# ut-vision/Rot-MVGaze

Measured on AMD Instinct MI355X. Metric: multi-view samples/sec (fwd+bwd), BxVx3x224x224, higher is better.
Workload: dtype f32; 1 GPU; C3: ResNet-50, V=4, B=128 per GPU, 3x224x224, fwd+loss+bwd; backbone=ResNet-50, views=4, batch_per_gpu=128, global_batch=128, image=3x224x224, parallelism=dp1, weights=random init, seed 0 (kaiming-normal convs, default Linear), rccl_ranks=1, step_launch=eager: every kernel queued from Python

## Files before the change

include/rotmvgaze.h:

```cpp
#ifndef ROTMVGAZE_H
#define ROTMVGAZE_H

#include <stddef.h>
#include <stdint.h>

#ifdef __cplusplus
extern "C" {
#endif

#define MVG_ABI_VERSION 13

int mvg_abi_version(void);
const char *mvg_last_error(void);
int mvg_device_cus(void);
int mvg_set_scratch(void *ptr, size_t bytes, void *stream);
size_t mvg_scratch_bytes(void);
void *mvg_stream_create_low_priority(void);
int mvg_set_reserved_cus(int n);

enum {
  MVG_K_CONV_FPROP = 0, MVG_K_CONV_DGRAD = 1, MVG_K_CONV_WGRAD = 2, MVG_K_WGRAD_REDUCE = 3,
  MVG_K_BN_FINALIZE = 4, MVG_K_BN_APPLY = 5, MVG_K_BN_BWD_REDUCE = 6, MVG_K_BN_BWD_APPLY = 7,
  MVG_K_POOL = 8, MVG_K_LAYOUT = 9, MVG_K_LINEAR_FPROP = 10, MVG_K_LINEAR_DGRAD = 11,
  MVG_K_LINEAR_WGRAD = 12, MVG_K_ROTCAT = 13, MVG_K_COLSUM = 14, MVG_K_LOSS = 15,
// ... 288 lines not shown
                                        int ho, int wo, float *s1, float *s2, float *dgamma, float *dbeta,
                                        int accumulate, float *workspace, void *stream);
int mvg_bn_relu_maxpool_bwd_apply_bf16(const uint16_t *g_pooled, const uint8_t *argmax, const uint16_t *y,
                                       const float *mean, const float *invstd, const float *gamma,
                                       const float *scale, const float *shift, const float *s1,
                                       const float *s2, int groups, int n_per_group, int h, int w, int c,
                                       int ho, int wo, uint16_t *dy, void *stream);
int mvg_bn_eval_bwd_bf16(const uint16_t *g, const uint16_t *act, const uint8_t *relu_bits, const uint16_t *y,
                         const float *relu_scale, const float *relu_shift, const float *gamma, const float *running_mean,
                         const float *running_var, float eps, int groups, int64_t rows_per_group, int c, uint16_t *dy,
                         uint16_t *dz_out, float *dgamma, float *dbeta, int accumulate, float *workspace, void *stream);
int mvg_bn_relu_maxpool_eval_bwd_bf16(const uint16_t *g_pooled, const uint8_t *argmax, const uint16_t *y, const float *scale,
                                      const float *shift, const float *gamma, const float *running_mean,
                                      const float *running_var, float eps, int groups, int n_per_group, int h, int w,
                                      int c, int ho, int wo, uint16_t *dy, float *dgamma, float *dbeta, int accumulate,
                                      float *workspace, void *stream);
int mvg_avgpool_fwd_bf16(const uint16_t *x, float *y, int n, int hw, int c, void *stream);
int mvg_avgpool_bwd_bf16(const float *dy, uint16_t *dx, int n, int hw, int c, void *stream);
int mvg_nchw_to_nhwc8_bf16(const float *src, uint16_t *dst, int n, int c, int h, int w, void *stream);
int mvg_preprocess_u8hwc_resize_bf16(const uint8_t *src, uint16_t *dst, int n, int h, int w, int oh, int ow, float mean0,
                                     float mean1, float mean2, float std0, float std1, float std2, int swap_rb,
                                     void *stream);

int mvg_split_f32(const float *x, void *out_sp, int64_t n, float scale, void *stream);
int mvg_merge_sp(const void *x_sp, float *out, int64_t n, float inv_scale, void *stream);
int mvg_split_weights(const mvg_conv_desc *d, const float *w, void *w_krsc_sp, void *w_crsk_sp, float *stat2, void *items_dev,
                      void *stream);
int mvg_weights_prep_batch(const void *items_dev, int n, int mode, int blocks_per_item , void *stream);
int mvg_conv_stats_partials_split(const mvg_conv_desc *d, int32_t *rows_per_partial);
int mvg_conv_fprop_split(const mvg_conv_desc *d, const void *x_sp, const float *x_sinv, const void *w_sp, const float *w_sinv,
                         float *y, float *stats, void *stream);
int mvg_conv_fprop_split_affine(const mvg_conv_desc *d, const void *x_sp, const float *x_sinv, const void *w_sp, const float *w_sinv,
                                void *out, int out_sp, const float *scale, const float *shift, const void *residual,
                                int residual_sp, int relu, void *stream);
int mvg_conv_fprop_split_affine_ranged(const mvg_conv_desc *d, const void *x_sp, const float *x_sinv, const void *w_sp,
                                       const float *w_sinv, void *out, int out_sp, const float *scale, const float *shift,
                                       const void *residual, int residual_sp, int relu, uint32_t *range_word, void *stream);
int mvg_split_f32_ranged(const float *x, void *out_sp, int64_t n, float scale, uint32_t *range_word, void *stream);
int mvg_conv_dgrad_split(const mvg_conv_desc *d, const void *dy_sp, const float *dy_sinv, const void *w_crsk_sp,
                         const float *w_sinv, float *dx, const float *addend, const void *relu_mask_sp, void *stream);
int mvg_bn_apply_split(const float *y, const float *scale, const float *shift, const void *residual, int residual_sp,
                       const float *res_scale, const float *res_shift, int relu, void *out_sp, uint8_t *relu_bits,
                       int groups, int64_t rows_per_group, int c, void *stream);
int mvg_bn_bwd_reduce_split(const float *g, const uint8_t *relu_bits, const float *y, const float *mean, const float *invstd,
                            const float *relu_scale, const float *relu_shift, int groups, int64_t rows_per_group, int c,
                            float *s1, float *s2, float *dgamma, float *dbeta, int accumulate, float *workspace,
                            float *dz_out, float *mx, const float *gamma, float *dy_sinv, void *stream);
int mvg_bn_bwd_apply_split(const float *g, const float *y, const float *mean, const float *invstd, const float *gamma,
                           const float *s1, const float *s2, const float *relu_scale, const float *relu_shift,
                           int groups, int64_t rows_per_group, int c, void *dy_sp, const float *mx, float *dy_sinv,
                           int dy_sinv_ready, void *stream);
int mvg_bn_relu_maxpool_fwd_split(const float *y, const float *scale, const float *shift, void *pooled_sp,
                                  uint8_t *argmax, int groups, int n_per_group, int h, int w, int c, int ho, int wo,
                                  void *stream);
int mvg_avgpool_fwd_split(const void *x_sp, float *y, int n, int hw, int c, void *stream);
int mvg_act_scales(const void *items_dev, int n, float *slots, int n_slots, void *stream);
int mvg_bn_apply_split_scaled(const float *y, const float *scale, const float *shift, const void *residual, int residual_sp,
                              const float *res_scale, const float *res_shift, const float *res_sinv, int relu, void *out_sp,
                              const float *out_sinv, uint8_t *relu_bits, int groups, int64_t rows_per_group, int c,
                              void *stream);
int mvg_bn_relu_maxpool_fwd_split_scaled(const float *y, const float *scale, const float *shift, void *pooled_sp,
                                         const float *pooled_sinv, uint8_t *argmax, int groups, int n_per_group, int h, int w,
                                         int c, int ho, int wo, void *stream);
int mvg_avgpool_fwd_split_scaled(const void *x_sp, const float *x_sinv, float *y, int n, int hw, int c, void *stream);
int mvg_conv_dgrad_bn_partials_split(const mvg_conv_desc *d);
int mvg_conv_dgrad_split_bnreduce(const mvg_conv_desc *d, const void *dy_sp, const float *dy_sinv, const void *w_crsk_sp,
                                  const float *w_sinv, float *dx, const float *addend, const float *bn_y, const uint8_t *bn_bits,
                                  const float *bn_mean, const float *bn_invstd, const float *relu_scale, const float *relu_shift,
                                  float *partials, float *s1, float *s2, float *dgamma, float *dbeta, int accumulate,
                                  float *mx, const float *bn_gamma, float *dx_dy_sinv, void *stream);
int mvg_conv_dgrad_split_bnapply_bnreduce(const mvg_conv_desc *d, void *dy_sp, const float *dy_sinv, const float *dz, const float *y,
                                          const float *mean, const float *invstd, const float *gamma, const float *un_s1,
                                          const float *un_s2, int64_t rows_per_group, const void *w_crsk_sp, const float *w_sinv,
                                          float *dx, const float *addend, const float *bn_y, const uint8_t *bn_bits,
                                          const float *bn_mean, const float *bn_invstd, const float *relu_scale,
                                          const float *relu_shift, float *partials, float *s1, float *s2, float *dgamma, float *dbeta,
                                          int accumulate, float *mx, const float *bn_gamma, float *dx_dy_sinv, void *stream);
int mvg_conv_fprop_split_stages(const mvg_conv_desc *d);
int mvg_conv_dgrad_split_stages(const mvg_conv_desc *d, int fused_reduce);
int mvg_conv_fprop_split_bnapply(const mvg_conv_desc *d, void *out_sp, const float *out_sinv, const float *bn_y, const float *scale,
                                 const float *shift, const void *residual, int residual_sp, const float *res_scale,
                                 const float *res_shift, const float *res_sinv, uint8_t *relu_bits, const void *w_sp,
                                 const float *w_sinv, float *y, float *stats, void *stream);
int mvg_stem_rowwindow_split(const float *x_nhwc4, void *xw_sp, int64_t images, int h, int w, void *stream);
int mvg_stem_rowwindow_split_nchw(const float *x_nchw, void *xw_sp, int64_t images, int h, int w, void *stream);
int mvg_stem_fprop_split(const mvg_conv_desc *d, const void *xw_sp, const void *w_sp, const float *w_sinv, float *y, float *stats,
                         void *stream);
int mvg_stem_wgrad_splits_split(const mvg_conv_desc *d);
int mvg_stem_wgrad_split(const mvg_conv_desc *d, const void *xw_sp, const void *dy_sp, const float *dy_sinv, float *dw_rw,
                         float *workspace, int splits, int accumulate, void *stream);
int mvg_bn_relu_maxpool_bwd_reduce_split(const float *g_pooled, const uint8_t *argmax, const float *y, const float *mean,
                                         const float *invstd, const float *scale, const float *shift, int groups,
                                         int n_per_group, int h, int w, int c, int ho, int wo, float *s1, float *s2,
                                         float *dgamma, float *dbeta, int accumulate, float *workspace, float *mx, const float *gamma,
                                         float *dy_sinv, void *stream);
int mvg_bn_relu_maxpool_bwd_apply_split(const float *g_pooled, const uint8_t *argmax, const float *y, const float *mean,
                                        const float *invstd, const float *gamma, const float *scale, const float *shift,
                                        const float *s1, const float *s2, int groups, int n_per_group, int h, int w, int c,
                                        int ho, int wo, void *dy_sp, const float *mx, float *dy_sinv, int dy_sinv_ready, void *stream);
int mvg_conv_wgrad_splits_split(const mvg_conv_desc *d);
int mvg_conv_wgrad_split_tile(const mvg_conv_desc *d, int32_t *bm, int32_t *bn, int32_t *incremental);
int mvg_conv_wgrad_split(const mvg_conv_desc *d, const void *x_sp, const void *dy_sp, const float *dy_sinv, float *dw,
                         float *workspace, int splits, int accumulate, void *stream);
int mvg_conv_wgrad_split_slabs(const mvg_conv_desc *d, const void *x_sp, const void *dy_sp, const float *dy_sinv, float *workspace,
                               int splits, void *stream);
int mvg_conv_wgrad_split_xs(const mvg_conv_desc *d, const void *x_sp, const float *x_sinv, const void *dy_sp, const float *dy_sinv,
                            float *dw, float *workspace, int splits, int accumulate, void *stream);
int mvg_conv_wgrad_split_slabs_xs(const mvg_conv_desc *d, const void *x_sp, const float *x_sinv, const void *dy_sp,
                                  const float *dy_sinv, float *workspace, int splits, void *stream);
int mvg_wgrad_reduce_batch(const float *const *host_slabs, float *const *host_dw, const int64_t *host_n, const int32_t *host_splits,
                           const int32_t *host_accumulate, int n, void *stream);

int mvg_absmax_multi(const float *const *host_ptrs, const int64_t *host_counts, float *const *host_out_slots, int n, void *stream);
int mvg_fuse_build_split(const float *img_feat, const float *feat, const float *rel, const int32_t *row_img, const int32_t *row_src_f,
                         const int32_t *row_src_h, void *xf_sp, void *xh_sp, const float *am_img, const float *am_feat,
                         float *xf_sinv, float *xh_sinv, int rows, int cf, int nvec, void *stream);
int mvg_fuse_unbuild(const float *dxh, const float *dxn, const float *rel, const int32_t *seg, const int32_t *vi, float *dfeat, float *da,
                     int da_accumulate, int segments, int views, int dirs, int batch, int cf, int nvec, float *absmax, void *stream);
int mvg_linear_fprop_split(int rows, int fin, int fout, const void *x_sp, const float *x_sinv, const void *w_sp, const float *w_sinv,
                           const float *bias, int relu, void *out, int out_sp, float *out_sinv, const float *bias_absmax,
                           float *out_absmax, void *stream);
int mvg_linear_dgrad_split(int rows, int fin, int fout, const void *dy_sp, const float *dy_sinv, const void *wt_sp, const float *w_sinv,
                           float *dx, const float *addend, const void *relu_mask_sp, float *out_absmax, void *stream);
int mvg_linear_wgrad_split(int rows, int fin, int fout, const void *x_sp, const float *x_sinv, const void *dy_sp, const float *dy_sinv,
                           float *dw, float *workspace, int splits, int accumulate, void *stream);
int mvg_split_colsum(const float *g, int rows, int cols, const float *absmax, void *out_sp, float *out_sinv, float *db, int accumulate,
                     void *stream);

typedef struct mvg_session mvg_session;
typedef struct {
  int32_t depth;
  int32_t num_iter;
  int32_t views, batch;
  int32_t height, width;
  int32_t share_weights, ignore_rotmat;
  int32_t split;
  int32_t raw_u8;
  int32_t in_h, in_w, input_bgr;
} mvg_session_cfg;

int mvg_session_create(const mvg_session_cfg *cfg, mvg_session **out);
#define MVG_SESSION_FP32 0
#define MVG_SESSION_BF16 1
int mvg_session_create_ex(const mvg_session_cfg *cfg, int32_t compute, mvg_session **out);
int mvg_session_compute(const mvg_session *s);
void mvg_session_destroy(mvg_session *s);
int mvg_session_num_tensors(const mvg_session *s);
const char *mvg_session_tensor_name(const mvg_session *s, int i);
int64_t mvg_session_tensor_numel(const mvg_session *s, int i);
size_t mvg_session_workspace_bytes(const mvg_session *s);
int mvg_session_launches(const mvg_session *s);
int mvg_session_num_steps(const mvg_session *s);
const char *mvg_session_step_name(const mvg_session *s, int i);
int mvg_session_bind(mvg_session *s, const void *const *host_tensor_ptrs, void *workspace, size_t bytes, void *stream);
int mvg_session_forward(mvg_session *s, const void *const *host_view_ptrs, const float *rot, float *img_feat, float *lifted,
                        float *feats, float *preds, void *stream);
int mvg_session_num_range_units(const mvg_session *s);
const char *mvg_session_range_unit_name(const mvg_session *s, int i);
int mvg_session_set_range_record(mvg_session *s, uint32_t *record_dev);

#ifdef __cplusplus
}
#endif
#endif
```

rot-mvgaze_amd/_lib.py:

```python
from __future__ import annotations

import ctypes as C
import os

_HERE = os.path.dirname(os.path.abspath(__file__))
LIB_PATH = os.path.join(_HERE, "csrc", "librotmvgaze_hip.so")

K_FAMILIES = 18
ABI_VERSION = 13
SESSION_FP32, SESSION_BF16 = 0, 1
ADAM_MAX_SEGMENTS = 16


class ConvDesc(C.Structure):
    _fields_ = [(n, C.c_int32) for n in
                ("groups", "n", "h", "w", "cin", "cout", "r", "s", "stride", "pad", "ho", "wo")]

    @classmethod
    def make(cls, groups, n, h, w, cin, cout, k, stride, pad):
        ho = (h + 2 * pad - k) // stride + 1
        wo = (w + 2 * pad - k) // stride + 1
        return cls(groups, n, h, w, cin, cout, k, k, stride, pad, ho, wo)

    @classmethod
# ... 25 lines not shown
                ("lanes_per_group", C.c_int32), ("slices", C.c_int32), ("partials_per_slice", C.c_int32), ("scratch_floats", C.c_int64)]


class ProfEntry(C.Structure):
    _fields_ = [("launches", C.c_int64), ("ms", C.c_double), ("flops", C.c_double), ("bytes", C.c_double)]


class SessionCfg(C.Structure):
    _fields_ = [(n, C.c_int32) for n in
                ("depth", "num_iter", "views", "batch", "height", "width", "share_weights", "ignore_rotmat", "split", "raw_u8",
                 "in_h", "in_w", "input_bgr")]


_P = C.c_void_p
_I = C.c_int
_I64 = C.c_int64
_F = C.c_float
_D = C.POINTER(ConvDesc)

SIGNATURES = {
    "mvg_abi_version": (_I, []),
    "mvg_last_error": (C.c_char_p, []),
    "mvg_device_cus": (_I, []),
    "mvg_set_scratch": (_I, [_P, C.c_size_t, _P]),
    "mvg_scratch_bytes": (C.c_size_t, []),
    "mvg_set_reserved_cus": (_I, [_I]),
    "mvg_stream_create_low_priority": (_P, []),
    "mvg_prof_enable": (_I, [_I]),
    "mvg_prof_reset": (_I, []),
    "mvg_prof_collect": (_I, [C.POINTER(ProfEntry)]),
    "mvg_prof_family_name": (C.c_char_p, [_I]),
    "mvg_conv_fprop": (_I, [_D, _P, _P, _P, _P, _I, _P, _P]),
    "mvg_conv_fprop_affine": (_I, [_D, _P, _P, _P, _P, _P, _P, _I, _P]),
    "mvg_conv_stats_partials": (_I, [_D, C.POINTER(C.c_int32)]),
    "mvg_conv_dgrad": (_I, [_D, _P, _P, _P, _P, _P, _P]),
    "mvg_conv_wgrad": (_I, [_D, _P, _P, _P, _P, _I, _I, _P]),
    "mvg_conv_wgrad_splits": (_I, [_D]),
    "mvg_conv_plan_query": (_I, [_D, _I, C.c_size_t, C.POINTER(ConvPlan)]),
    "mvg_bn_plan_query": (_I, [_I, _I, _I, _I64, _I, _I, _I, _I, _I, C.c_size_t, C.POINTER(BnPlan)]),
    "mvg_conv_wgrad_tile": (_I, [_D, C.POINTER(C.c_int32), C.POINTER(C.c_int32), C.POINTER(C.c_int32)]),
    "mvg_linear_wgrad": (_I, [_P, _P, _P, _P, _I, _I, _I, _P, _I, _I, _P]),
    "mvg_fuser_fprop": (_I, [_P, _P, _P, _P, _P, _P, _P, _I, _P, _I, _I, _I, _I, _I, _I, _P, C.c_size_t, _P]),
    "mvg_fuser_wgrad": (_I, [_P, _P, _P, _P, _P, _P, _P, _P, _I, _I, _I, _I, _I, _I, _P, _I, _I, _P]),
    "mvg_linear_workspace_floats": (C.c_size_t, [_I, _I, _I]),
    "mvg_linear_fprop": (_I, [_P, _P, _P, _I, _P, _I, _I, _I, _P, C.c_size_t, _P]),
    "mvg_linear_dgrad": (_I, [_P, _P, _P, _P, _P, _I, _I, _I, _P, C.c_size_t, _P]),
    "mvg_bn_finalize": (_I, [_P, _I, _I, _I, _I64, _I, _P, _P, _P, _P, _F, _F, _P, _P, _P, _P, _P]),
    "mvg_bn_eval_affine": (_I, [_I, _I, _P, _P, _P, _P, _F, _P, _P, _P]),
    "mvg_bn_eval_affine_batch": (_I, [_P, _I, _I, _F, _P]),
    "mvg_bn_apply": (_I, [_P, _P, _P, _P, _P, _P, _I, _P, _I, _I64, _I, _P]),
    "mvg_bn_bwd_reduce": (_I, [_P, _P, _P, _P, _P, _P, _P, _I, _I64, _I, _P, _P, _P, _P, _I, _P, _P, _P]),
    "mvg_split_f32": (_I, [_P, _P, _I64, _F, _P]),
    "mvg_merge_sp": (_I, [_P, _P, _I64, _F, _P]),
    "mvg_split_weights": (_I, [_D, _P, _P, _P, _P, _P, _P]),
    "mvg_weights_prep_batch": (_I, [_P, _I, _I, _I, _P]),
    "mvg_conv_stats_partials_split": (_I, [_D, C.POINTER(C.c_int32)]),
    "mvg_conv_fprop_split": (_I, [_D, _P, _P, _P, _P, _P, _P, _P]),
    "mvg_conv_fprop_split_affine": (_I, [_D, _P, _P, _P, _P, _P, _I, _P, _P, _P, _I, _I, _P]),
    "mvg_conv_dgrad_split": (_I, [_D, _P, _P, _P, _P, _P, _P, _P, _P]),
    "mvg_bn_apply_split": (_I, [_P, _P, _P, _P, _I, _P, _P, _I, _P, _P, _I, _I64, _I, _P]),
    "mvg_bn_bwd_apply_split": (_I, [_P, _P, _P, _P, _P, _P, _P, _P, _P, _I, _I64, _I, _P, _P, _P, _I, _P]),
    "mvg_bn_bwd_reduce_split": (_I, [_P, _P, _P, _P, _P, _P, _P, _I, _I64, _I, _P, _P, _P, _P, _I, _P, _P, _P, _P, _P, _P]),
    "mvg_bn_relu_maxpool_fwd_split": (_I, [_P, _P, _P, _P, _P, _I, _I, _I, _I, _I, _I, _I, _P]),
    "mvg_avgpool_fwd_split": (_I, [_P, _P, _I, _I, _I, _P]),
    "mvg_act_scales": (_I, [_P, _I, _P, _I, _P]),
    "mvg_bn_apply_split_scaled": (_I, [_P, _P, _P, _P, _I, _P, _P, _P, _I, _P, _P, _P, _I, _I64, _I, _P]),
    "mvg_bn_relu_maxpool_fwd_split_scaled": (_I, [_P, _P, _P, _P, _P, _P, _I, _I, _I, _I, _I, _I, _I, _P]),
    "mvg_avgpool_fwd_split_scaled": (_I, [_P, _P, _P, _I, _I, _I, _P]),
    "mvg_conv_wgrad_split_xs": (_I, [_D, _P, _P, _P, _P, _P, _P, _I, _I, _P]),
    "mvg_conv_wgrad_split_slabs_xs": (_I, [_D, _P, _P, _P, _P, _P, _I, _P]),
    "mvg_stem_rowwindow_split": (_I, [_P, _P, _I64, _I, _I, _P]),
    "mvg_stem_rowwindow_split_nchw": (_I, [_P, _P, _I64, _I, _I, _P]),
    "mvg_stem_fprop_split": (_I, [_D, _P, _P, _P, _P, _P, _P]),
    "mvg_stem_wgrad_splits_split": (_I, [_D]),
    "mvg_stem_wgrad_split": (_I, [_D, _P, _P, _P, _P, _P, _I, _I, _P]),
    "mvg_bn_relu_maxpool_bwd_reduce_split": (_I, [_P, _P, _P, _P, _P, _P, _P, _I, _I, _I, _I, _I, _I, _I, _P, _P, _P, _P, _I, _P, _P, _P, _P, _P]),
    "mvg_bn_relu_maxpool_bwd_apply_split": (_I, [_P, _P, _P, _P, _P, _P, _P, _P, _P, _P, _I, _I, _I, _I, _I, _I, _I, _P, _P, _P, _I, _P]),
    "mvg_conv_dgrad_bn_partials_split": (_I, [_D]),
    "mvg_conv_dgrad_split_bnreduce": (_I, [_D, _P, _P, _P, _P, _P, _P, _P, _P, _P, _P, _P, _P, _P, _P, _P, _P, _P, _I, _P, _P, _P, _P]),
    "mvg_conv_dgrad_split_bnapply_bnreduce": (_I, [_D] + [_P] * 9 + [_I64] + [_P] * 15 + [_I, _P, _P, _P, _P]),
    "mvg_conv_fprop_split_stages": (_I, [_D]),
    "mvg_conv_dgrad_split_stages": (_I, [_D, _I]),
    "mvg_conv_fprop_split_bnapply": (_I, [_D] + [_P] * 6 + [_I] + [_P] * 9),
    "mvg_conv_wgrad_splits_split": (_I, [_D]),
    "mvg_conv_wgrad_split_tile": (_I, [_D, C.POINTER(C.c_int32), C.POINTER(C.c_int32), C.POINTER(C.c_int32)]),
    "mvg_conv_wgrad_split": (_I, [_D, _P, _P, _P, _P, _P, _I, _I, _P]),
    "mvg_conv_wgrad_split_slabs": (_I, [_D, _P, _P, _P, _P, _I, _P]),
    "mvg_wgrad_reduce_batch": (_I, [C.POINTER(C.c_void_p), C.POINTER(C.c_void_p), C.POINTER(C.c_int64), C.POINTER(C.c_int32),
                                    C.POINTER(C.c_int32), _I, _P]),
    "mvg_bn_apply_bits": (_I, [_P, _P, _P, _P, _P, _P, _P, _P, _I, _I64, _I, _P]),
    "mvg_bn_bwd_reduce_bits": (_I, [_P, _P, _P, _P, _P, _I, _I64, _I, _P, _P, _P, _P, _I, _P, _P, _P]),
    "mvg_bn_apply_bits_bf16": (_I, [_P, _P, _P, _P, _P, _P, _P, _P, _I, _I64, _I, _P]),
    "mvg_bn_bwd_reduce_bits_bf16": (_I, [_P, _P, _P, _P, _P, _I, _I64, _I, _P, _P, _P, _P, _I, _P, _P, _P]),
    "mvg_bn_bwd_workspace_floats": (C.c_size_t, [_I, _I64, _I]),
    "mvg_bn_bwd_apply": (_I, [_P, _P, _P, _P, _P, _P, _P, _P, _P, _P, _I, _I64, _I, _P, _P, _P]),
    "mvg_maxpool3x3s2_fwd": (_I, [_P, _P, _P, _I, _I, _I, _I, _I, _I, _P]),
    "mvg_maxpool3x3s2_bwd": (_I, [_P, _P, _P, _I, _I, _I, _I, _I, _I, _P]),
    "mvg_bn_relu_maxpool_fwd": (_I, [_P, _P, _P, _P, _P, _I, _I, _I, _I, _I, _I, _I, _P]),
    "mvg_bn_relu_maxpool_bwd_reduce": (_I, [_P, _P, _P, _P, _P, _P, _P, _I, _I, _I, _I, _I, _I, _I, _P, _P, _P, _P, _I, _P,
                                            _P]),
    "mvg_bn_relu_maxpool_bwd_apply": (_I, [_P, _P, _P, _P, _P, _P, _P, _P, _P, _P, _I, _I, _I, _I, _I, _I, _I, _P, _P]),
    "mvg_bn_eval_bwd": (_I, [_P, _P, _P, _P, _P, _P, _P, _P, _P, _F, _I, _I64, _I, _P, _P, _P, _P, _I, _P, _P]),
    "mvg_bn_eval_bwd_workspace_floats": (C.c_size_t, [_I, _I64, _I]),
    "mvg_bn_relu_maxpool_eval_bwd": (_I, [_P, _P, _P, _P, _P, _P, _P, _P, _F, _I, _I, _I, _I, _I, _I, _I, _P, _P, _P, _I, _P,
                                          _P]),
    "mvg_avgpool_fwd": (_I, [_P, _P, _I, _I, _I, _P]),
    "mvg_avgpool_bwd": (_I, [_P, _P, _I, _I, _I, _P]),
    "mvg_nchw_to_nhwc4": (_I, [_P, _P, _I, _I, _I, _I, _P]),
    "mvg_nhwc4_to_nchw": (_I, [_P, _P, _I, _I, _I, _I, _P]),
    "mvg_preprocess_u8hwc": (_I, [_P, _P, _I, _I, _I, _F, _F, _F, _F, _F, _F, _I, _P]),
    "mvg_gaze_lp_loss": (_I, [_P, _P, _I, _I, _P, _P, _P]),
    "mvg_preprocess_u8hwc_resize": (_I, [_P, _P, _I, _I, _I, _I, _I, _F, _F, _F, _F, _F, _F, _I, _P]),
    "mvg_multi_erase_nchw": (_I, [_P, _P, _P, _I, _I, _I, _I, _I, _P]),
    "mvg_augment_u8hwc": (_I, [_P, _P, _P, _P, _P, _P, _P, _I, _I, _I, _I, _F, _F, _F, _F, _F, _F, _I, _P]),
    "mvg_augment_u8hwc_bf16": (_I, [_P, _P, _P, _P, _P, _P, _P, _I, _I, _I, _I, _F, _F, _F, _F, _F, _F, _I, _P]),
    "mvg_rotation_matrix_2d": (_I, [_P, _P, _I, _I, _P]),
    "mvg_relative_rotation": (_I, [_P, _P, _P, _P, _I, _I, _I, _P]),
    "mvg_rotcat_fwd": (_I, [_P, _P, _P, _P, _P, _P, _I, _I, _I, _I, _P]),
    "mvg_rotcat_bwd": (_I, [_P, _P, _P, _P, _I, _I, _I, _I, _P]),
    "mvg_rotcat_ext_fwd": (_I, [_P, _P, _P, _P, _P, _P, _P, _I, _I, _I, _I, _I, _P]),
    "mvg_rotcat_ext_bwd": (_I, [_P, _I, _P, _P, _P, _I, _I, _I, _I, _P]),
    "mvg_ibn_scales": (_I, [_P, _P, _P, _P, _P, _I, _F, _F, _P, _I, _I, _I, _P]),
    "mvg_paircat_fwd": (_I, [_P, _P, _P, _P, _P, _P, _P, _I, _I, _I, _P]),
    "mvg_paircat_bwd": (_I, [_P, _P, _P, _P, _P, _P, _I, _I, _I, _P]),
    "mvg_segment_sum": (_I, [_P, _I64, _I, _P, _P, _I, _I, _I, _I, _P]),
    "mvg_axpby": (_I, [_P, _P, _F, _F, _I64, _P]),
    "mvg_scale_by": (_I, [_P, _P, _P, _I64, _P]),
    "mvg_linear_skinny_fwd": (_I, [_P, _P, _P, _P, _I, _I, _I, _P]),
    "mvg_linear_skinny_bwd": (_I, [_P, _P, _P, _P, _P, _P, _P, _I, _I, _I, _I, _P, _P]),
    "mvg_adam_step": (_I, [_P, _P, _P, _P, _I64, _F, _F, _F, _F, _F, _I, _P]),
    "mvg_gaze_angular_loss": (_I, [_P, _P, _I, _F, _P, _I, _P, _P, _P]),
    "mvg_gaze_angular_loss_multi": (_I, [_P, _P, _I, _I, _I, C.POINTER(C.c_float), _P, _P, _P]),
    "mvg_adam_step_dev": (_I, [_P, _P, _P, _P, _I64, _P, _P, _F, _F, _F, _F, _P]),
    "mvg_adam_step_segments": (_I, [_P, _P, _P, _P, _I64, C.POINTER(C.c_int64), C.POINTER(C.c_float), C.POINTER(C.c_int32), _I, _P]),
    "mvg_adam_step_segments_dev": (_I, [_P, _P, _P, _P, _I64, C.POINTER(C.c_int64), C.POINTER(C.c_float), C.POINTER(C.c_int32), _I, _P, _I, _P,
                                        _P]),
    "mvg_absmax_multi": (_I, [C.POINTER(C.c_void_p), C.POINTER(C.c_int64), C.POINTER(C.c_void_p), _I, _P]),
    "mvg_fuse_build_split": (_I, [_P, _P, _P, _P, _P, _P, _P, _P, _P, _P, _P, _P, _I, _I, _I, _P]),
    "mvg_fuse_unbuild": (_I, [_P, _P, _P, _P, _P, _P, _P, _I, _I, _I, _I, _I, _I, _I, _P, _P]),
    "mvg_linear_fprop_split": (_I, [_I, _I, _I, _P, _P, _P, _P, _P, _I, _P, _I, _P, _P, _P, _P]),
    "mvg_linear_dgrad_split": (_I, [_I, _I, _I, _P, _P, _P, _P, _P, _P, _P, _P, _P]),
    "mvg_linear_wgrad_split": (_I, [_I, _I, _I, _P, _P, _P, _P, _P, _P, _I, _I, _P]),
    "mvg_split_colsum": (_I, [_P, _I, _I, _P, _P, _P, _P, _I, _P]),
    "mvg_cast_weights_bf16": (_I, [_D, _P, _I, _P, _P, _P]),
    "mvg_conv_fprop_bf16": (_I, [_D, _P, _P, _P, _P, _I, _P, _P]),
    "mvg_conv_stats_partials_bf16": (_I, [_D, C.POINTER(C.c_int32)]),
    "mvg_conv_fprop_bf16_affine": (_I, [_D, _P, _P, _P, _P, _P, _P, _I, _P]),
    "mvg_conv_dgrad_bf16": (_I, [_D, _P, _P, _P, _P, _P, _P]),
    "mvg_conv_dgrad_bn_partials_bf16": (_I, [_D]),
    "mvg_conv_dgrad_bf16_bnreduce": (_I, [_D, _P, _P, _P, _P, _P, _P, _P, _P, _P, _P, _P, _P, _P, _P, _P, _I, _P]),
    "mvg_conv_wgrad_bf16": (_I, [_D, _P, _P, _P, _P, _I, _I, _P]),
    "mvg_stem_rowwindow_bf16": (_I, [_P, _P, _I64, _I, _I, _P]),
    "mvg_stem_fprop_bf16": (_I, [_D, _P, _P, _P, _P, _P]),
    "mvg_stem_wgrad_splits_bf16": (_I, [_D]),
    "mvg_stem_wgrad_bf16": (_I, [_D, _P, _P, _P, _P, _I, _I, _P]),
    "mvg_conv_wgrad_splits_bf16": (_I, [_D]),
    "mvg_conv_wgrad_bf16_slabs": (_I, [_D, _P, _P, _P, _I, _P]),
    "mvg_conv_plan_query_bf16": (_I, [_D, _I, C.POINTER(ConvPlan)]),
    "mvg_conv_wgrad_tile_bf16": (_I, [_D, _I, C.POINTER(C.c_int32), C.POINTER(C.c_int32), C.POINTER(C.c_int32)]),
    "mvg_linear_fprop_mixed": (_I, [_P, _P, _P, _I, _P, _I, _I, _I, _P]),
    "mvg_linear_dgrad_mixed": (_I, [_P, _P, _P, _P, _P, _I, _I, _I, _P]),
    "mvg_linear_wgrad_mixed": (_I, [_P, _P, _P, _P, _I, _I, _I, _P, _I, _I, _P]),
    "mvg_bn_apply_bf16": (_I, [_P, _P, _P, _P, _P, _P, _I, _P, _I, _I64, _I, _P]),
    "mvg_bn_bwd_reduce_bf16": (_I, [_P, _P, _P, _P, _P, _P, _P, _I, _I64, _I, _P, _P, _P, _P, _I, _P, _P, _P]),
    "mvg_bn_bwd_apply_bf16": (_I, [_P, _P, _P, _P, _P, _P, _P, _P, _P, _P, _I, _I64, _I, _P, _P, _P]),
    "mvg_bn_relu_maxpool_fwd_bf16": (_I, [_P, _P, _P, _P, _P, _I, _I, _I, _I, _I, _I, _I, _P]),
# ... 62 lines not shown
```

rot-mvgaze_amd/backbone.py:

```python
from __future__ import annotations

import enum
import math
import os
from dataclasses import dataclass
from typing import Callable, Dict, List, NamedTuple, Optional

import numpy as np
import torch

from . import ops
from ._lib import ConvDesc
from .arch import RANGE_OVER_BITS, BackboneSpec, ConvSpec, backbone_spec, range_unit_names

Tensor = torch.Tensor
BN_EPS, BN_MOMENTUM = 1e-5, 0.1
IMAGE_MEAN, IMAGE_STD = (0.485, 0.456, 0.406), (0.229, 0.224, 0.225)


BN_APPLY_DGRAD_MAX_COUT = 512


def bn_apply_dgrad_eligible(c: ConvSpec, *, split: bool, trained: bool, fused_in: bool, carries_reduce: bool,
                            need_dimg: bool = False) -> bool:
    return bool(split and trained and not need_dimg and fused_in and carries_reduce
                and c.k == 1 and c.stride == 1 and c.pad == 0 and c.cin in (64, 128)
                and c.cout % 32 == 0 and c.cout <= BN_APPLY_DGRAD_MAX_COUT)


def bn_apply_dgrad_units(spec: BackboneSpec, *, split: bool = True, bf16: bool = False, training: bool = True,
                         need_dimg: bool = False, fuse_bn_split: bool = True, enabled: bool = True) -> List[str]:
    on = enabled and split and not bf16 and fuse_bn_split
    nb = len(spec.blocks)
    return [blk.convs[-1].name for bi, blk in reversed(list(enumerate(spec.blocks)))
            if bn_apply_dgrad_eligible(blk.convs[-1], split=on, trained=training, fused_in=bi < nb - 1,
                                       carries_reduce=len(blk.convs) > 1, need_dimg=need_dimg)]


BN_APPLY_FPROP_MAX_CIN = 512


def bn_apply_fprop_eligible(producer: ConvSpec, consumer: ConvSpec, *, split: bool, trained: bool, residual: bool = True,
                            relu: bool = True, single_stage: bool = True) -> bool:
    return bool(split and trained and residual and relu and single_stage
                and consumer.k == 1 and consumer.stride == 1 and consumer.pad == 0 and consumer.cout in (64, 128)
                and consumer.cin == producer.cout and consumer.cin % 32 == 0 and consumer.cin <= BN_APPLY_FPROP_MAX_CIN)


def bn_apply_fprop_pairs(spec: BackboneSpec, *, split: bool = True, bf16: bool = False, training: bool = True, enabled: bool = True,
                         single_stage: Optional[Callable[[ConvSpec], bool]] = None) -> List[tuple]:
    on = enabled and split and not bf16
    return [(a.convs[-1].name, b.convs[0].name) for a, b in zip(spec.blocks[:-1], spec.blocks[1:])
            if bn_apply_fprop_eligible(a.convs[-1], b.convs[0], split=on, trained=training,
                                       single_stage=True if single_stage is None else single_stage(b.convs[0]))]


class GradSink:

    def view(self, p: torch.nn.Parameter) -> Tensor:
        raise NotImplementedError

    def wants(self, p: torch.nn.Parameter) -> bool:
        return True

    def accumulate(self, p: torch.nn.Parameter) -> bool:
        raise NotImplementedError

    def publish(self, ps: List[torch.nn.Parameter]) -> None:
        raise NotImplementedError


class Family(enum.Enum):
    FP32 = 0
    SPLIT = 1
    BF16 = 2


class Call(NamedTuple):
    V: int
    B: int
    H: int
    W: int
    training: bool
    keep_tape: bool
    bf16: bool
    split: bool
    sp: bool
    stem_rw: bool
    taped: bool
    guard: Optional[str]
    range_live: bool
    need_dimg: bool
    boundary: int
    wprep: Optional[Dict[str, tuple]] = None
    act_sinv: Optional[Dict[str, Tensor]] = None
    train_step: Optional[bool] = None


def plan_call(spec: BackboneSpec, *, V: int, B: int, H: int, W: int, training: bool, keep_tape: bool, raw: bool = False,
              augment: bool = False, need_dimg: bool = False, boundary: int = -1, bf16: bool = False, split: bool = True,
              split_eval: bool = True, split_eval_guard: Optional[str] = None, stem_rowwindow: bool = True,
              batch_weight_prep: bool = True, bf16_fold_eval: bool = True, guard_scale: int = 1, tripped: bool = False,
              capturing: bool = False, train_step: Optional[bool] = None) -> Call:
    step = training if train_step is None else bool(train_step)
    if bf16 and raw and (step or keep_tape) and not (step and augment):
        raise NotImplementedError("raw uint8 input with the bf16 path is served for inference only (model.eval() under "
                                  "torch.no_grad()) and for training steps with model.input_augment (augment.TrainAugment; the "
                                  "identity augment for un-augmented steps): else normalise to fp32 NCHW first")
    biggest_view_elems = B * ((H + 3) // 4) * ((W + 3) // 4) * spec.blocks[0].convs[-1].cout
    split = split and 4 * biggest_view_elems * guard_scale < 0x7FFFFFF0
    infer = not (training or keep_tape or bf16)
    if split_eval_guard not in (None, "record", "fallback"):
        raise ValueError(f"split_eval_guard must be None, 'record' or 'fallback' (got {split_eval_guard!r})")
    guard = split_eval_guard if infer else None
    if guard == "fallback" and capturing:
        raise RuntimeError("split_eval_guard = 'fallback' reads the range record on the host and cannot run while the stream "
                           "is capturing: capture with 'record' and check overflowed() after the replay")
    if guard == "fallback" and tripped:
        split = False
    if bf16:
        ho, wo = (H - 1) // 2 + 1, W // 2
        stem_rw = (stem_rowwindow and training and W % 4 == 0 and (B * ho * (wo // 2)) % 64 == 0 and batch_weight_prep
                   and spec.stem.k == 7)
    else:
        stem_rw = (split and stem_rowwindow and training and not need_dimg and W % 2 == 0
                   and batch_weight_prep and 32 * B * H * (W // 2) * 4 < 0x7FFFFFF0)
    taped = training or keep_tape or (bf16 and not bf16_fold_eval)
    sp = split and not bf16 and (training or (infer and split_eval))
    return Call(V, B, H, W, training, keep_tape, bf16, split, sp, stem_rw, taped, guard,
                range_live=guard is not None and sp, need_dimg=need_dimg, boundary=boundary, train_step=step)


def unit_family(call: Call, c: ConvSpec) -> Family:
    if call.bf16:
        return Family.BF16
    if call.sp and (c.cin != 3 or call.stem_rw):
        return Family.SPLIT
    return Family.FP32


class _Apply(NamedTuple):
    y: Tensor
    scale: Tensor
    shift: Tensor
    residual: Optional[Tensor]
    residual_affine: Optional[tuple]
    bits: Optional[Tensor]


class _PendingDy(NamedTuple):
    dz: Tensor
    s1: Tensor
    s2: Tensor


class _FusedSums(NamedTuple):
    s1: Tensor
    s2: Tensor
    mx: Optional[Tensor] = None
    sinv: Optional[Tensor] = None


class _Pool(NamedTuple):
    argmax: Tensor
    scale: Tensor
    shift: Tensor
    ho: int
    wo: int
    hp: int
    wp: int


@dataclass(slots=True)
class _Unit:
    spec: Optional[ConvSpec] = None
    desc: Optional[ConvDesc] = None
    x_in: Optional[Tensor] = None
    y: Optional[Tensor] = None
    out: Optional[Tensor] = None
    mean: Optional[Tensor] = None
    invstd: Optional[Tensor] = None
    relu: bool = False
    rows: int = 0
    w: Optional[Tensor] = None
    trained: bool = True
    pool: Optional[_Pool] = None
    relu_affine: Optional[tuple] = None
    fused_s12: Optional[_FusedSums] = None
    relu_bits: Optional[Tensor] = None
    family: Family = Family.FP32
    stem_rw: bool = False


class _Fwd(NamedTuple):
    out: Tensor
    affine: Optional[tuple] = None
    pending: Optional[_Apply] = None


class Backbone:
    _guard_scale = 1
    _debug_units: Optional[list] = None

    def __init__(self, depth: int, params: Dict[str, Tensor], prefix: str = "_feat_extractor.0."):
        self.spec: BackboneSpec = backbone_spec(depth, prefix)
        self.p = params
        self.fc_dim = self.spec.fc_dim
        self.overlap_wgrad = True
        self.overlap_head = True
        self.wgrad_low_priority = True
        self.grad_streams: List[torch.cuda.Stream] = []
        self._wg_stream: Optional[torch.cuda.Stream] = None
        self._wg_low = True
        self.act_dtype = torch.float32
        self.relu_bits = True
        self.split = os.environ.get("MVG_SPLIT", "1") != "0"
        self.fuse_bn_split = True
        self.fuse_bn_apply_dgrad = True
        self.fuse_bn_apply_fprop = True
        self.stem_rowwindow = True
        self.split_eval = True
        self.split_eval_guard: Optional[str] = None
        self._range_record: Optional[Tensor] = None
        self._range_slot: Dict[str, int] = {n: i for i, n in enumerate(range_unit_names(depth, prefix))}
        self._range_tripped = False
        self.bf16_fold_eval = True
        self._wprep_infer_ok = False
        self._wk_cache: Dict[str, tuple] = {}
        self.batch_weight_prep = True
        self._wprep_state = None
        self._wprep_versions = None
        self._ascale_state = None
        self._wg_defer: Optional[list] = None
        self._last_call: Optional[Call] = None
        self._stem_w8 = None

    @property
    def bf16(self) -> bool:
        return self.act_dtype == torch.bfloat16

    @property
    def _split_now(self) -> bool:
        return self._last_call.split if self._last_call is not None else self.split

    @property
    def _stem_rw(self) -> bool:
        return self._last_call is not None and self._last_call.stem_rw

    @property
    def _act_sinv(self) -> Optional[Dict[str, Tensor]]:
        return self._last_call.act_sinv if self._last_call is not None else None

    def _prepare_weights(self, dev, family: Family, stem_rw: bool, reuse: bool = False) -> Dict[str, tuple]:
        mode = 0 if family is Family.BF16 else 1
        convs = [c for c in self.spec.all_convs() if not (mode == 1 and c.cin == 3 and not stem_rw)]
        key = (mode, stem_rw, str(dev), tuple(self.p[c.name + ".weight"].data_ptr() for c in convs))
        if self._wprep_state is None or self._wprep_state[0] != key:
            out, rows = {}, []
            wstat = torch.zeros(len(convs), 2, dtype=torch.float32, device=dev)
            self._stem_w8 = None
            for ci, c in enumerate(convs):
                wsrc = self.p[c.name + ".weight"]
                assert wsrc.is_contiguous(memory_format=torch.channels_last) or (c.k == 1 and wsrc.is_contiguous())
                rs = c.k * c.k
                if mode == 1 and c.cin == 3:
                    assert c.k == 7
                    self._stem_w8 = torch.zeros(c.cout, 7, 8, 4, dtype=torch.float32, device=dev)
                    wk = ops.sp_empty(c.cout, 7 * 32, device=dev)
                    wk.sinv = wstat[ci, 1:2]
                    out[c.name] = (wk, None)
                    rows.append([self._stem_w8.data_ptr(), wk.data_ptr(), 0, c.cout | (7 << 32), 32 | (32 << 32), wstat[ci].data_ptr()])
                    continue
                if mode == 0 and c.cin == 3 and stem_rw:
                    assert c.k == 7
                    self._stem_w8 = torch.zeros(2 * c.cout, 7, 16, 4, dtype=torch.float32, device=dev)
                    wk = torch.empty(2 * c.cout, 7, 1, 64, dtype=torch.bfloat16, device=dev)
                    out[c.name] = (wk, None)
                    rows.append([self._stem_w8.data_ptr(), wk.data_ptr(), 0, (2 * c.cout) | (7 << 32), 64 | (64 << 32), wstat[ci].data_ptr()])
                    continue
                if mode == 1:
                    wk = ops.sp_empty(c.cout, rs * c.cin, device=dev)
                    wt = ops.sp_empty(c.cin, rs * c.cout, device=dev)
                    wk.sinv = wt.sinv = wstat[ci, 1:2]
                    cin_pad = c.cin
                else:
                    cin_pad = 8 if c.cin == 3 else c.cin
                    wk = torch.empty(c.cout, c.k, c.k, cin_pad, dtype=torch.bfloat16, device=dev)
                    wt = None if c.cin == 3 else torch.empty(cin_pad, c.k, c.k, c.cout, dtype=torch.bfloat16, device=dev)
                out[c.name] = (wk, wt)
                rows.append([wsrc.data_ptr(), wk.data_ptr(), wt.data_ptr() if wt is not None else 0, c.cout | (rs << 32),
                             c.cin | (cin_pad << 32), wstat[ci].data_ptr()])
            table = torch.tensor(rows, dtype=torch.int64).to(dev)
            self._wprep_state = (key, out, table, len(rows), mode, wstat)
        elif (reuse and self._wprep_infer_ok and
              self._wprep_versions == tuple(self.p[c.name + ".weight"]._version for c in self.spec.all_convs())):
            return self._wprep_state[1]
        _, out, table, n, mode, wstat = self._wprep_state
        self._wprep_infer_ok = reuse
        if mode == 1:
            wstat.zero_()
            if self._stem_w8 is not None:
                self._stem_w8[:, :, 1:, :3].copy_(self.p[self.spec.stem.name + ".weight"].detach().permute(0, 2, 3, 1))
# ... 118 lines not shown
                self._debug_units.append((c.name, x, residual, y))
            return y
        ops.conv_fprop_affine(d, x, w, y, scale, shift, residual, relu)
        if not pool:
            return y
        pooled = self._pool_plain(y, G, N, d.ho, d.wo, c.cout)
        if call.range_live:
            return ops.split_f32_ranged(pooled, self._range_word(c))
        return ops.split_f32(pooled) if call.sp else pooled

    def _range_word(self, c: ConvSpec) -> Tensor:
        i = self._range_slot[c.name]
        return self._range_record[i:i + 1]

    @staticmethod
    def _pool_plain(a0: Tensor, G: int, N: int, h: int, w: int, c: int) -> Tensor:
        hp, wp_ = (h + 2 - 3) // 2 + 1, (w + 2 - 3) // 2 + 1
        x = torch.empty(G, N, hp, wp_, c, dtype=torch.float32, device=a0.device)
        argmax = torch.empty(G, N, hp, wp_, c, dtype=torch.uint8, device=a0.device)
        ops.maxpool_fwd(a0, x, argmax, G * N, h, w, c, hp, wp_)
        return x

    @staticmethod
    def _stats_partials(c: ConvSpec, d: ConvDesc, family: Family, stem_rw: bool):
        if family is Family.BF16:
            if stem_rw:
                P, rpp = ops.conv_stats_partials(ConvDesc.make(d.groups, d.n, d.ho, d.wo // 2, 64, 2 * c.cout, 1, 1, 0), True)
                return 2 * P, rpp
            return ops.conv_stats_partials(d, True)
        if family is Family.SPLIT:
            if stem_rw:
                return ops.conv_stats_partials_split(ConvDesc.make(d.groups, d.n, d.ho, d.wo, 32, c.cout, 1, 1, 0))
            return ops.conv_stats_partials_split(d)
        return ops.conv_stats_partials(d, False)

    def _unit_fwd(self, call: Call, c: ConvSpec, x: Tensor, H: int, W: int, *, relu: bool, residual: Optional[Tensor] = None,
                  tape: Optional[list] = None, pool: bool = False, residual_affine=None, defer_apply: bool = False,
                  next_conv: Optional[ConvSpec] = None, pending_apply: Optional[_Apply] = None) -> _Fwd:
        family = unit_family(call, c)
        stem_rw = c.cin == 3 and call.stem_rw
        G, N, training, keep = call.V, call.B, call.training, tape is not None
        d = ConvDesc.make(G, N, H, W, (8 if family is Family.BF16 else 4) if c.cin == 3 else c.cin, c.cout, c.k, c.stride, c.pad)
        assert pending_apply is None or (family is Family.SPLIT and not stem_rw)
        assert not stem_rw or call.wprep is not None
        w, w_t = self._conv_weights(call, c, d, family, keep)
        rows = N * d.ho * d.wo
        partials = self._stats_partials(c, d, family, stem_rw) if training else None
        y, stats = self._conv_fwd(c, d, family, stem_rw, x, w, pending_apply, partials)
        mean, invstd, scale, shift = self._bn_fwd_stats(c, G, rows, stats, partials)
        out = bits = pool_rec = handed = None
        if defer_apply:
            assert not relu and residual is None and not pool
        elif pool:
            assert relu and residual is None
            out, pool_rec = self._stem_tail(call, c, d, y, scale, shift)
            if self._debug_units is not None and not keep and not training:
                self._debug_units.append((c.name, x, y, out))
        else:
            out, bits, handed = self._apply_fwd(call, c, d, family, y, scale, shift, relu, residual, residual_affine, keep, next_conv)
        if keep:
            tape.append(_Unit(spec=c, desc=d, x_in=x, y=y, out=None if pool else out, mean=mean, invstd=invstd, relu=relu,
                              rows=rows, w=w if family is Family.FP32 else w_t, trained=training, family=family, stem_rw=stem_rw,
                              relu_affine=(scale, shift) if (relu and residual is None and not pool) else None,
                              pool=pool_rec, relu_bits=bits))
        return _Fwd(y, affine=(scale, shift)) if defer_apply else _Fwd(out, pending=handed)

    def _conv_fwd(self, c: ConvSpec, d: ConvDesc, family: Family, stem_rw: bool, x: Tensor, w: Tensor,
                  pending_apply: Optional[_Apply], partials: Optional[tuple]):
        dev = x.device
        y = torch.empty(d.groups, d.n, d.ho, d.wo, c.cout, dtype=self.act_dtype, device=dev)
        stats = None
        if partials is not None:
            stats = torch.empty(d.groups, partials[0], 2, c.cout, dtype=torch.float32, device=dev)
        if family is Family.BF16:
            if stem_rw:
                ops.stem_fprop_bf16(d, x, w, y, stats)
            else:
                ops.conv_fprop(d, x, w, y, None, False, stats)
        elif family is Family.SPLIT:
            if stem_rw:
                ops.stem_fprop_split(d, x, w, y, stats)
            elif pending_apply is not None:
                p = pending_apply
                ops.conv_fprop_split_bnapply(d, x, p.y, p.scale, p.shift, p.residual, w, y, stats, p.residual_affine, p.bits)
            else:
                ops.conv_fprop_split(d, x, w, y, stats)
        else:
            ops.conv_fprop(d, x, w, y, None, False, stats)
        return y, stats

    def _bn_fwd_stats(self, c: ConvSpec, G: int, rows: int, stats: Optional[Tensor], partials: Optional[tuple]):
        gamma, beta = self.p[c.bn + ".weight"].detach(), self.p[c.bn + ".bias"].detach()
        rm, rv = self.p[c.bn + ".running_mean"], self.p[c.bn + ".running_var"]
        mean, invstd, scale, shift = torch.empty(4, G, c.cout, dtype=torch.float32, device=gamma.device)
        if partials is not None:
            P, rpp = partials
            ops.bn_finalize(stats, G, P, rpp, rows, c.cout, gamma, beta, rm, rv, BN_MOMENTUM, BN_EPS, mean, invstd,
                            scale, shift)
        else:
            ops.bn_eval_affine(G, c.cout, gamma, beta, rm, rv, BN_EPS, scale, shift)
        return mean, invstd, scale, shift

    def _apply_fwd(self, call: Call, c: ConvSpec, d: ConvDesc, family: Family, y: Tensor, scale: Tensor, shift: Tensor, relu: bool,
                   residual: Optional[Tensor], residual_affine, keep: bool, next_conv: Optional[ConvSpec]):
        G, rows = d.groups, d.n * d.ho * d.wo
        if call.sp:
            out = ops.sp_empty(G, d.n, d.ho, d.wo, c.cout, device=y.device)
            out.sinv = call.act_sinv[c.name]
            want_bits = keep and relu and residual is not None
            if (next_conv is not None and self.fuse_bn_apply_fprop
                    and bn_apply_fprop_eligible(c, next_conv, split=family is Family.SPLIT, trained=call.training,
                                                residual=residual is not None, relu=relu)
                    and ops.conv_fprop_split_stages(ConvDesc.make(G, d.n, d.ho, d.wo, next_conv.cin, next_conv.cout, 1, 1, 0)) == 1):
                bits = torch.empty(G * rows * c.cout // 4, dtype=torch.uint8, device=y.device) if want_bits else None
                return out, bits, _Apply(y, scale, shift, residual, residual_affine, bits)
            bits = ops.bn_apply_split(y, scale, shift, residual, relu, out, G, rows, c.cout, residual_affine, want_bits=want_bits)
            return out, bits, None
        out = torch.empty_like(y) if keep else y
        if keep and relu and residual is not None and self.relu_bits:
            return out, ops.bn_apply_bits(y, scale, shift, residual, out, G, rows, c.cout, residual_affine), None
        ops.bn_apply(y, scale, shift, residual, relu, out, G, rows, c.cout, residual_affine)
        return out, None, None

    def _stem_tail(self, call: Call, c: ConvSpec, d: ConvDesc, y: Tensor, scale: Tensor, shift: Tensor):
        G, N = y.shape[0], y.shape[1]
        hp, wp_ = (d.ho + 2 - 3) // 2 + 1, (d.wo + 2 - 3) // 2 + 1
        argmax = torch.empty(G, N, hp, wp_, c.cout, dtype=torch.uint8, device=y.device)
        if call.sp:
            out = ops.sp_empty(G, N, hp, wp_, c.cout, device=y.device)
            out.sinv = call.act_sinv[c.name]
            ops.bn_relu_maxpool_fwd_split(y, scale, shift, out, argmax, G, N, d.ho, d.wo, c.cout, hp, wp_)
        else:
            out = torch.empty(G, N, hp, wp_, c.cout, dtype=self.act_dtype, device=y.device)
            ops.bn_relu_maxpool_fwd(y, scale, shift, out, argmax, G, N, d.ho, d.wo, c.cout, hp, wp_)
        return out, _Pool(argmax, scale, shift, d.ho, d.wo, hp, wp_)

    def _input_layout(self, call: Call, imgs: List[Tensor], input_bgr: bool, augment=None) -> Tensor:
        V, B, H, W, dev, bf = call.V, call.B, call.H, call.W, imgs[0].device, call.bf16
        raw = imgs[0].dtype == torch.uint8
        direct = call.stem_rw and (not raw or (bf and augment is not None))
        if direct and bf:
            x0 = torch.empty(V, B, H, W // 4, 64, dtype=self.act_dtype, device=dev)
        elif direct:
            x0 = ops.sp_empty(V, B, H, W // 2, 32, device=dev)
            x0.sinv = None
        else:
            x0 = torch.empty(V, B, H, W, 8 if bf else 4, dtype=self.act_dtype, device=dev)
        for v, im in enumerate(imgs):
            assert im.shape == imgs[0].shape and im.is_cuda and im.dtype == imgs[0].dtype
            if raw and augment is not None:
                if tuple(im.shape[1:3]) != (H, W):
                    raise ValueError(f"input_augment: {im.shape[1]} x {im.shape[2]} patches with input_size {H} x {W}: a resize "
                                     "after the augmentation is not served (set model.input_size = None, or feed patches of that size)")
                if torch.cuda.is_current_stream_capturing():
                    raise RuntimeError("input_augment draws on the host for every step and cannot be captured (graph.GraphedStep): "
                                       "augment outside the captured step (TrainAugment.apply) and feed the result")
                if bf and direct:
                    augment.launch(im, augment.draw(B, H, W), None, None, input_bgr, dst_rw=x0[v])
                elif bf:
                    augment.launch(im, augment.draw(B, H, W), None, None, input_bgr, dst_nhwc8=x0[v])
                else:
                    augment.launch(im, augment.draw(B, H, W), None, x0[v], input_bgr)
                continue
            if raw:
                prep = ops.preprocess_u8hwc_resize_bf16 if bf else ops.preprocess_u8hwc_resize
                prep(im.contiguous(), x0[v], B, im.shape[1], im.shape[2], H, W, IMAGE_MEAN, IMAGE_STD, input_bgr)
                continue
            assert im.dtype == torch.float32
            if direct:
                (ops.stem_rowwindow_bf16 if bf else ops.stem_rowwindow_split_nchw)(im.detach().contiguous(), x0[v])
            else:
                (ops.nchw_to_nhwc8_bf16 if bf else ops.nchw_to_nhwc4)(im.detach().contiguous(), x0[v], B, 3, H, W)
        if call.stem_rw and not direct:
            x0 = ops.stem_rowwindow_split(x0)
        return x0

    def forward(self, imgs: List[Tensor], training: bool, keep_tape: bool, input_bgr: bool = False,
                input_size: Optional[int] = None, need_dimg: bool = False, input_augment=None,
                train_step: Optional[bool] = None):
        step = training if train_step is None else bool(train_step)
        V = len(imgs)
        raw = imgs[0].dtype == torch.uint8
        if raw:
            B, Hin, Win, C = imgs[0].shape
            H, W = (input_size, input_size) if input_size else (Hin, Win)
        else:
            B, C, H, W = imgs[0].shape
        assert C == 3
        dev = imgs[0].device
        call = plan_call(self.spec, V=V, B=B, H=H, W=W, training=training, keep_tape=keep_tape, raw=raw,
                         augment=input_augment is not None, need_dimg=need_dimg, boundary=self._boundary(need_dimg) if keep_tape else -1,
                         bf16=self.bf16, split=self.split, split_eval=self.split_eval, split_eval_guard=self.split_eval_guard,
                         stem_rowwindow=self.stem_rowwindow, batch_weight_prep=self.batch_weight_prep,
                         bf16_fold_eval=self.bf16_fold_eval, guard_scale=self._guard_scale, tripped=self._range_tripped,
                         capturing=self.split_eval_guard == "fallback" and torch.cuda.is_current_stream_capturing(),
                         train_step=step)
        x0 = self._input_layout(call, imgs, input_bgr, input_augment if (raw and step) else None)
        if step:
# ... 398 lines not shown
```

rot-mvgaze_amd/csrc/bf16_tile.h:

```cpp
#pragma once
#include "conv_shared.h"
#include "bn_math.h"
#include "elem.h"

namespace mvg {

typedef __bf16 bf16x8 __attribute__((ext_vector_type(8)));
typedef short s16x4 __attribute__((ext_vector_type(4)));

__device__ __forceinline__ float bf_lo(unsigned v) { return __uint_as_float(v << 16); }
__device__ __forceinline__ float bf_hi(unsigned v) { return __uint_as_float(v & 0xFFFF0000u); }
__device__ __forceinline__ unsigned pack_bf2(float a, float b) {
  const __bf16 x = (__bf16)a, y = (__bf16)b;
  return (unsigned)__builtin_bit_cast(unsigned short, x) | ((unsigned)__builtin_bit_cast(unsigned short, y) << 16);
}

__device__ __forceinline__ void ld8(const float *p, float (&v)[8]) {
  const float4 a = *reinterpret_cast<const float4 *>(p), b = *reinterpret_cast<const float4 *>(p + 4);
  v[0] = a.x; v[1] = a.y; v[2] = a.z; v[3] = a.w; v[4] = b.x; v[5] = b.y; v[6] = b.z; v[7] = b.w;
}

constexpr unsigned RANGE_OVER_BITS = 0x477FF000u;
__device__ __forceinline__ unsigned range_bits(unsigned mx, float v) {
  const unsigned b = __float_as_uint(v) & 0x7FFFFFFFu;
  return b > mx ? b : mx;
}
__device__ __forceinline__ void range_commit(unsigned mx, unsigned *lds, unsigned *__restrict__ word, int tid) {
#pragma unroll
  for (int o = 32; o > 0; o >>= 1) {
    const unsigned other = (unsigned)__shfl_xor((int)mx, o, 64);
    mx = other > mx ? other : mx;
  }
  __syncthreads();
  if ((tid & 63) == 0) lds[tid >> 6] = mx;
  __syncthreads();
  if (tid == 0) {
    unsigned m = lds[0];
    for (int k = 1; k < 4; ++k) m = lds[k] > m ? lds[k] : m;
    if (m > *word) atomicMax(word, m);
  }
}

template <int BM, int BN, int PASSES, bool BNF, bool AFF = false>
constexpr int bf16_epilogue_bytes() {
  return (BM / PASSES) * (BN + 4) * 4 + BM * 4 + (BNF ? 4 * BN * 4 : 0) + (AFF ? 2 * BN * 4 : 0);
}

template <int BM, int BN, int WGM, bool DGRAD, bool F32IO, int PASSES = 1, bool ACC16 = false, bool BNF = false, bool LIN = false, int WGN = 2,
          bool AFF = false, bool RNG = false, class AccT>
__device__ __forceinline__ void bf16_epilogue(const IgemmParams &p, const IgemmClass &c, AccT &acc,
                                              unsigned short *smem, int tid, int g, int mtile, int ntile) {
  constexpr int NT = WGM * WGN * 64;
  constexpr int WTM = BM / WGM, WTN = BN / WGN;
  constexpr int TS = ACC16 ? 16 : 32, NE = ACC16 ? 4 : 16;
  constexpr int TM = WTM / TS, TN = WTN / TS;
  constexpr int LDO = BN + 4;
  const int lane = tid & 63, wave = tid >> 6;
  const int wm = wave / WGN, wn = wave % WGN;
  const int li = ACC16 ? (lane & 15) : (lane & 31), lh = ACC16 ? (lane >> 4) : (lane >> 5);
  auto erow = [&](int e) { return ACC16 ? 4 * lh + e : (e & 3) + 8 * (e >> 2) + 4 * lh; };
  const int ohw = c.out_h * c.out_w;
  const long long row_base = (long long)mtile * BM + wm * WTM;
  const float osc = F32IO ? (p.a_sinv ? *p.a_sinv : 1.f) * (p.b_sinv ? *p.b_sinv : 1.f) : 1.f;
  float lin_scale = 1.f, lin_max = 0.f;
  unsigned rng_max = 0u;
  static_assert(!RNG || (F32IO && !DGRAD && !LIN && !BNF && !AFF && WGM * WGN == 4), "bf16_epilogue: RNG is a forward form of the split conv kernels");
  if constexpr (LIN && F32IO) {
    if (!DGRAD && p.out_sp && p.out_sinv) {
      const float bound = (float)p.ktotal * 1073741824.f * osc + (p.bias_absmax ? *p.bias_absmax : 0.f);
      lin_scale = sp_scale_for(bound);
      if (tid == 0 && mtile == 0 && ntile == 0 && g == 0) *p.out_sinv = 1.f / lin_scale;
    }
  }
  if (!DGRAD && !AFF && p.stats) {
    long long cnt_ll = c.rows_per_group - row_base;
    const int cnt = cnt_ll <= 0 ? 0 : (cnt_ll > WTM ? WTM : (int)cnt_ll);
#pragma unroll
    for (int j = 0; j < TN; ++j) {
      const int col = ntile * BN + wn * WTN + j * TS + li;
      float csum = 0.f;
#pragma unroll
      for (int i = 0; i < TM; ++i)
#pragma unroll
        for (int e = 0; e < NE; ++e) {
          const int r = i * TS + erow(e);
          csum += (r < cnt) ? acc[i][j][e] : 0.f;
        }
      csum += __shfl_xor(csum, 32, 64);
      if (ACC16) csum += __shfl_xor(csum, 16, 64);
      const float mean = cnt > 0 ? csum / (float)cnt : 0.f;
      float q = 0.f;
#pragma unroll
      for (int i = 0; i < TM; ++i)
#pragma unroll
        for (int e = 0; e < NE; ++e) {
          const int r = i * TS + erow(e);
          const float dlt = acc[i][j][e] - mean;
          q += (r < cnt) ? dlt * dlt : 0.f;
        }
      q += __shfl_xor(q, 32, 64);
      if (ACC16) q += __shfl_xor(q, 16, 64);
      long long P = p.stats_partials ? p.stats_partials : (long long)c.mtiles_per_group * WGM;
      long long pi = (long long)mtile * WGM + wm;
      if (lh == 0 && col < p.ncols && (pi < P || p.stats_fold)) {
        int nc = p.ncols, ch = col;
        if (p.stats_fold) {
          nc = p.ncols >> 1;
          pi = 2 * pi + (col >= nc);
          ch = col - (col >= nc ? nc : 0);
          P *= 2;
        }
        float *st = p.stats + (((long long)g * P + pi) * 2) * nc;
        st[ch] = csum * osc;
        st[nc + ch] = q * (osc * osc);
      }
    }
  }
  static_assert(WGM % PASSES == 0, "bf16_epilogue: the wave rows must divide into the passes");
  constexpr int PR = BM / PASSES;
  float *ot = reinterpret_cast<float *>(smem);
  int *rowoff = reinterpret_cast<int *>(ot + PR * LDO);
  for (int r = tid; r < BM; r += NT) {
    const long long m = (long long)mtile * BM + r;
    int off = -1;
    if (m < c.rows_per_group) {
      if (DGRAD && p.cls_step == 2) {
        const int rr = (int)m;
        const int img = (int)fdiv((unsigned)rr, c.ohw_div), rem = rr - img * ohw;
        const int y2 = (int)fdiv((unsigned)rem, c.ow_div), x2 = rem - y2 * c.out_w;
        off = ((img * p.full_h + 2 * y2 + c.cls_py) * p.full_w + 2 * x2 + c.cls_px) * p.ncols;
      } else {
        off = (int)m * p.ncols;
      }
    }
    rowoff[r] = off;
  }
  const long long gelems = DGRAD ? (long long)p.imgs_per_group * p.full_h * p.full_w * p.ncols
                                 : c.rows_per_group * (long long)p.ncols;
  unsigned short *out_g = reinterpret_cast<unsigned short *>(p.out) + (long long)g * gelems;
  const unsigned short *add_g = p.addend ? reinterpret_cast<const unsigned short *>(p.addend) + (long long)g * gelems : nullptr;
  const unsigned short *mask_g = p.mask ? reinterpret_cast<const unsigned short *>(p.mask) + (long long)g * gelems : nullptr;
  float *out_f = p.out + (long long)g * gelems;
  const float *add_f = p.addend ? p.addend + (long long)g * gelems : nullptr;
  const float *mask_f = p.mask ? p.mask + (long long)g * gelems : nullptr;
  constexpr int CV = BN / 8;
  const bool bnf = BNF && DGRAD && p.bn_part != nullptr;
  bool quad = false;
  if constexpr (F32IO && DGRAD && !LIN) quad = !p.mask && (p.ncols % BN) == 0;
  float bn_s1[8], bn_s2[8], bn_mx[8];
  const bool bn_aff = bnf && p.bn_rscale != nullptr;
  float *bnc = reinterpret_cast<float *>(smem) + (BM / PASSES) * LDO + BM;
  if (bnf) {
    for (int cc = tid; cc < BN; cc += NT) {
      const int colc = ntile * BN + cc;
      const bool ok = colc < p.ncols;
      bnc[cc] = ok ? p.bn_mean[(long long)g * p.ncols + colc] : 0.f;
      bnc[BN + cc] = ok ? p.bn_invstd[(long long)g * p.ncols + colc] : 0.f;
      bnc[2 * BN + cc] = (ok && bn_aff) ? p.bn_rscale[(long long)g * p.ncols + colc] : 0.f;
      bnc[3 * BN + cc] = (ok && bn_aff) ? p.bn_rshift[(long long)g * p.ncols + colc] : 0.f;
    }
#pragma unroll
    for (int k = 0; k < 8; ++k) bn_s1[k] = bn_s2[k] = bn_mx[k] = 0.f;
  }
  float *affc = reinterpret_cast<float *>(smem) + (BM / PASSES) * LDO + BM;
  if constexpr (AFF) {
    static_assert(!DGRAD && !F32IO && !BNF && !LIN, "bf16_epilogue: AFF is the forward form of the bf16 storage kernels");
    for (int cc = tid; cc < BN; cc += NT) {
      const int colc = ntile * BN + cc;
      const bool ok = colc < p.ncols;
      affc[cc] = ok ? p.scale[colc] : 0.f;
      affc[BN + cc] = ok ? p.bias[colc] : 0.f;
    }
  }
#pragma unroll
  for (int ph = 0; ph < PASSES; ++ph) {
  if (PASSES > 1 && ph > 0) __syncthreads();
  if (wm / (WGM / PASSES) == ph) {
#pragma unroll
    for (int i = 0; i < TM; ++i)
#pragma unroll
      for (int j = 0; j < TN; ++j)
#pragma unroll
        for (int e = 0; e < NE; ++e)
          ot[((wm % (WGM / PASSES)) * WTM + i * TS + erow(e)) * LDO + wn * WTN + j * TS + li] = acc[i][j][e];
  }
  __syncthreads();
  auto store_rows = [&](int it) {
    const int v = tid + it * NT;
    const int rl = v / CV, cv = v - rl * CV;
    const int r = ph * PR + rl;
    const int col = ntile * BN + cv * 8;
    const int off = rowoff[r];
    if (off < 0 || col >= p.ncols) return;
    const float4 lo = *reinterpret_cast<const float4 *>(ot + rl * LDO + cv * 8);
    const float4 hi = *reinterpret_cast<const float4 *>(ot + rl * LDO + cv * 8 + 4);
    float x[8] = {lo.x, lo.y, lo.z, lo.w, hi.x, hi.y, hi.z, hi.w};
    if constexpr (F32IO) {
#pragma unroll
      for (int k = 0; k < 8; ++k) x[k] *= osc;
    }
    if constexpr (AFF) {
      asm volatile("" ::: "memory");
      float sa[8], sb[8];
      ld8(affc + cv * 8, sa);
      ld8(affc + BN + cv * 8, sb);
#pragma unroll
      for (int k = 0; k < 8; ++k) x[k] = __builtin_fmaf(x[k], sa[k], sb[k]);
      if (add_g) {
        const u32x4 a = *reinterpret_cast<const u32x4 *>(add_g + off + col);
        const unsigned aa[4] = {a.x, a.y, a.z, a.w};
#pragma unroll
        for (int k = 0; k < 4; ++k) {
          x[2 * k] += bf_lo(aa[k]);
          x[2 * k + 1] += bf_hi(aa[k]);
        }
      }
      if (p.relu) {
#pragma unroll
        for (int k = 0; k < 8; ++k) x[k] = fmaxf(x[k], 0.f);
      }
      u32x4 o;
      o.x = pack_bf2(x[0], x[1]);
      o.y = pack_bf2(x[2], x[3]);
      o.z = pack_bf2(x[4], x[5]);
      o.w = pack_bf2(x[6], x[7]);
      *reinterpret_cast<u32x4 *>(out_g + off + col) = o;
      return;
    }
    if (!DGRAD && F32IO && p.scale) {
      const float4 s0 = *reinterpret_cast<const float4 *>(p.scale + col), s1 = *reinterpret_cast<const float4 *>(p.scale + col + 4);
      x[0] *= s0.x; x[1] *= s0.y; x[2] *= s0.z; x[3] *= s0.w; x[4] *= s1.x; x[5] *= s1.y; x[6] *= s1.z; x[7] *= s1.w;
    }
    if (!DGRAD && p.bias) {
      const float4 b0 = *reinterpret_cast<const float4 *>(p.bias + col), b1 = *reinterpret_cast<const float4 *>(p.bias + col + 4);
      x[0] += b0.x; x[1] += b0.y; x[2] += b0.z; x[3] += b0.w; x[4] += b1.x; x[5] += b1.y; x[6] += b1.z; x[7] += b1.w;
    }
    if (!DGRAD && p.relu && !(F32IO && p.addend)) {
#pragma unroll
      for (int k = 0; k < 8; ++k) x[k] = fmaxf(x[k], 0.f);
    }
    if constexpr (F32IO) {
      if (!DGRAD && p.addend) {
        if (p.addend_sp) {
          const uint4 *q = reinterpret_cast<const uint4 *>(p.addend) + (((long long)g * gelems + off + col) >> 3) * SP_NP;
          float r[8];
          merge2_chunk(q[0], q[1], r);
#pragma unroll
          for (int k = 0; k < 8; ++k) x[k] += r[k];
        } else {
          const float4 a0 = *reinterpret_cast<const float4 *>(add_f + off + col), a1 = *reinterpret_cast<const float4 *>(add_f + off + col + 4);
          x[0] += a0.x; x[1] += a0.y; x[2] += a0.z; x[3] += a0.w; x[4] += a1.x; x[5] += a1.y; x[6] += a1.z; x[7] += a1.w;
        }
        if (p.relu) {
#pragma unroll
          for (int k = 0; k < 8; ++k) x[k] = fmaxf(x[k], 0.f);
        }
      }
      if (!DGRAD && p.out_sp) {
        if constexpr (LIN) {
#pragma unroll
          for (int k = 0; k < 8; ++k) x[k] *= lin_scale;
        }
        if constexpr (RNG) {
#pragma unroll
          for (int k = 0; k < 8; ++k) rng_max = range_bits(rng_max, x[k]);
        }
        uint4 q1, q2;
        split2_chunk(x, q1, q2);
        uint4 *dst = reinterpret_cast<uint4 *>(p.out) + (((long long)g * gelems + off + col) >> 3) * SP_NP;
        dst[0] = q1;
        dst[1] = q2;
        return;
      }
      if (DGRAD && mask_f) {
// ... 95 lines not shown
      for (int k = 0; k < 4; ++k) {
        const float y0 = bf_lo(yw[k]), y1 = bf_hi(yw[k]);
        const bool on0 = ((bits >> (2 * k)) & 1u) != 0u, on1 = ((bits >> (2 * k + 1)) & 1u) != 0u;
        ow[k] = pack_bf2(on0 ? x[2 * k] : 0.f, on1 ? x[2 * k + 1] : 0.f);
        const float d0 = bf_lo(ow[k]), d1 = bf_hi(ow[k]);
        bn_s1[2 * k] += d0;
        bn_s1[2 * k + 1] += d1;
        bn_s2[2 * k] = __builtin_fmaf(d0, y0, bn_s2[2 * k]);
        bn_s2[2 * k + 1] = __builtin_fmaf(d1, y1, bn_s2[2 * k + 1]);
      }
      o.x = ow[0]; o.y = ow[1]; o.z = ow[2]; o.w = ow[3];
    } else {
      o.x = pack_bf2(x[0], x[1]);
      o.y = pack_bf2(x[2], x[3]);
      o.z = pack_bf2(x[4], x[5]);
      o.w = pack_bf2(x[6], x[7]);
    }
    *reinterpret_cast<u32x4 *>(out_g + off + col) = o;
  };
  if (quad) {
    constexpr int HB = BN / 2;
    const int cq = tid % CV;
    const int cA = cq * 4, cB = HB + cq * 4;
    const int colA = ntile * BN + cA, colB = ntile * BN + cB;
#pragma unroll 1
    for (int it = 0; it < PR * CV / NT; ++it) {
      const int rl = (tid + it * NT) / CV;
      const int off = rowoff[ph * PR + rl];
      if (off < 0) continue;
      const float4 qa = *reinterpret_cast<const float4 *>(ot + rl * LDO + cA);
      const float4 qb = *reinterpret_cast<const float4 *>(ot + rl * LDO + cB);
      float x[8] = {qa.x * osc, qa.y * osc, qa.z * osc, qa.w * osc, qb.x * osc, qb.y * osc, qb.z * osc, qb.w * osc};
      if (add_f) {
        const float4 a0 = *reinterpret_cast<const float4 *>(add_f + off + colA), a1 = *reinterpret_cast<const float4 *>(add_f + off + colB);
        x[0] += a0.x; x[1] += a0.y; x[2] += a0.z; x[3] += a0.w; x[4] += a1.x; x[5] += a1.y; x[6] += a1.z; x[7] += a1.w;
      }
      if (bnf) {
        const float *yg = p.bn_y + (long long)g * gelems + off;
        const float4 y0 = *reinterpret_cast<const float4 *>(yg + colA), y1 = *reinterpret_cast<const float4 *>(yg + colB);
        const float yy[8] = {y0.x, y0.y, y0.z, y0.w, y1.x, y1.y, y1.z, y1.w};
        unsigned bits = 0xFFu;
        if (p.bn_bits) {
          const uint8_t *bb = p.bn_bits + (((long long)g * gelems + off) >> 2);
          bits = (bb[colA >> 2] & 0xFu) | ((bb[colB >> 2] & 0xFu) << 4);
        }
        asm volatile("" ::: "memory");
        auto ld44 = [&](const float *base, float (&v)[8]) {
          const float4 u = *reinterpret_cast<const float4 *>(base + cA), w = *reinterpret_cast<const float4 *>(base + cB);
          v[0] = u.x; v[1] = u.y; v[2] = u.z; v[3] = u.w; v[4] = w.x; v[5] = w.y; v[6] = w.z; v[7] = w.w;
        };
        if (bn_aff) {
          float bn_ra[8], bn_rb[8];
          ld44(bnc + 2 * BN, bn_ra);
          ld44(bnc + 3 * BN, bn_rb);
#pragma unroll
          for (int k = 0; k < 8; ++k) bits = (bits & ~(1u << k)) | ((relu_on(yy[k], bn_ra[k], bn_rb[k]) ? 1u : 0u) << k);
        }
        float bn_mu[8], bn_is[8];
        ld44(bnc, bn_mu);
        ld44(bnc + BN, bn_is);
#pragma unroll
        for (int k = 0; k < 8; ++k) {
          x[k] = ((bits >> k) & 1u) != 0u ? x[k] : 0.f;
          bn_mx[k] = fmaxf(bn_mx[k], fabsf(x[k]));
          bn_s1[k] += x[k];
          bn_s2[k] += x[k] * xhat(yy[k], bn_mu[k], bn_is[k]);
        }
      }
      if (p.nt_out) {
        typedef float f4v __attribute__((ext_vector_type(4)));
        const f4v s0 = {x[0], x[1], x[2], x[3]}, s1 = {x[4], x[5], x[6], x[7]};
        __builtin_nontemporal_store(s0, reinterpret_cast<f4v *>(out_f + off + colA));
        __builtin_nontemporal_store(s1, reinterpret_cast<f4v *>(out_f + off + colB));
      } else {
        *reinterpret_cast<float4 *>(out_f + off + colA) = make_float4(x[0], x[1], x[2], x[3]);
        *reinterpret_cast<float4 *>(out_f + off + colB) = make_float4(x[4], x[5], x[6], x[7]);
      }
    }
    continue;
  }
  bool plain4 = false;
  if constexpr (F32IO && !LIN) plain4 = p.nt_out && !p.scale && !p.bias && !p.addend && !p.mask && !p.out_sp && !bnf && !p.relu;
  if (plain4) {
    constexpr int CV4 = BN / 4;
#pragma unroll
    for (int it = 0; it < PR * CV4 / NT; ++it) {
      const int v = tid + it * NT;
      const int rl = v / CV4, c4 = v - rl * CV4;
      const int col = ntile * BN + c4 * 4;
      const int off = rowoff[ph * PR + rl];
      if (off < 0 || col >= p.ncols) continue;
      const float4 q = *reinterpret_cast<const float4 *>(ot + rl * LDO + c4 * 4);
      typedef float f4v __attribute__((ext_vector_type(4)));
      const f4v sv = {q.x * osc, q.y * osc, q.z * osc, q.w * osc};
      __builtin_nontemporal_store(sv, reinterpret_cast<f4v *>(out_f + off + col));
    }
  } else if constexpr (BNF) {
#pragma unroll 1
    for (int it = 0; it < PR * CV / NT; ++it) store_rows(it);
  } else {
#pragma unroll
    for (int it = 0; it < PR * CV / NT; ++it) store_rows(it);
  }
  }
  if constexpr (RNG) range_commit(rng_max, reinterpret_cast<unsigned *>(smem), p.out_absmax, tid);
  if constexpr (LIN && F32IO) {
    if (p.out_absmax) {
#pragma unroll
      for (int o = 32; o > 0; o >>= 1) lin_max = fmaxf(lin_max, __shfl_xor(lin_max, o, 64));
      __syncthreads();
      float *wred = reinterpret_cast<float *>(smem);
      if (lane == 0) wred[wave] = lin_max;
      __syncthreads();
      if (tid == 0) {
        float mx = wred[0];
        for (int k = 1; k < NT / 64; ++k) mx = fmaxf(mx, wred[k]);
        if (mx > 0.f) atomicMax(p.out_absmax, __float_as_uint(mx));
      }
      __syncthreads();
    }
  }
  if (bnf) {
    constexpr int RL = NT / CV;
    __syncthreads();
    float *red = reinterpret_cast<float *>(smem);
    const int cvt = tid % CV, rlt = tid / CV;
    const int nred = p.bn_part_rows;
#pragma unroll
    for (int k = 0; k < 8; ++k) {
      const int cc = quad ? (k < 4 ? cvt * 4 + k : BN / 2 + cvt * 4 + k - 4) : cvt * 8 + k;
      red[(0 * RL + rlt) * BN + cc] = bn_s1[k];
      red[(1 * RL + rlt) * BN + cc] = bn_s2[k];
      if (F32IO) red[(2 * RL + rlt) * BN + cc] = bn_mx[k];
    }
    __syncthreads();
    for (int idx = tid; idx < nred * BN; idx += NT) {
      const int which = idx / BN, cc = idx - which * BN;
      const int colr = ntile * BN + cc;
      if (colr >= p.ncols) continue;
      float t = 0.f;
      if (which < 2)
        for (int r = 0; r < RL; ++r) t += red[(which * RL + r) * BN + cc];
      else
        for (int r = 0; r < RL; ++r) t = fmaxf(t, red[(which * RL + r) * BN + cc]);
      p.bn_part[(((long long)g * p.bn_parts + c.part0 + mtile) * nred + which) * p.ncols + colr] = t;
    }
  }
}

__device__ __forceinline__ bf16x8 tr_frag(const unsigned short *img, int ld, int k0, int m0, int lane) {
  const int t = lane & 15, q = t >> 2, pq = t & 3;
  const int mh = (lane >> 4) & 1, kh = lane >> 5;
  const unsigned short *a = img + (k0 + 8 * kh + q) * ld + m0 + 16 * mh + 4 * pq;
  typedef s16x4 __attribute__((address_space(3))) * lds_p;
  const s16x4 x = __builtin_amdgcn_ds_read_tr16_b64_v4i16((lds_p)(a));
  const s16x4 y = __builtin_amdgcn_ds_read_tr16_b64_v4i16((lds_p)(a + 4 * ld));
  typedef short s16x8 __attribute__((ext_vector_type(8)));
  const s16x8 z = {x[0], x[1], x[2], x[3], y[0], y[1], y[2], y[3]};
  return __builtin_bit_cast(bf16x8, z);
}

}
```

rot-mvgaze_amd/csrc/conv_split.hip:

```cpp
#include "bf16_tile.h"
#include "elem.h"

namespace mvg {

typedef _Float16 f16x8 __attribute__((ext_vector_type(8)));

#define SPLIT_ONE(PA, PB, av, bv, acc)                                                                         \
  _Pragma("unroll") for (int i = 0; i < TM; ++i) _Pragma("unroll") for (int j = 0; j < TN; ++j)                \
      acc[i][j] = __builtin_amdgcn_mfma_f32_32x32x16_f16(av[PA][i], bv[PB][j], acc[i][j], 0, 0, 0);
#define SPLIT_PRODUCTS(av, bv, acc) SPLIT_ONE(0, 1, av, bv, acc) SPLIT_ONE(1, 0, av, bv, acc) SPLIT_ONE(0, 0, av, bv, acc)

constexpr int SP_BM = 128, SP_BK = 32;

__global__ __launch_bounds__(256) void split_f32_kernel(const float4 *__restrict__ x, uint4 *__restrict__ out, long long n8, float scale) {
  const long long stride = (long long)gridDim.x * 256;
  for (long long i = (long long)blockIdx.x * 256 + threadIdx.x; i < n8; i += stride) {
    const float4 lo = x[2 * i], hi = x[2 * i + 1];
    const float v[8] = {lo.x * scale, lo.y * scale, lo.z * scale, lo.w * scale, hi.x * scale, hi.y * scale, hi.z * scale, hi.w * scale};
    uint4 q1, q2;
    split2_chunk(v, q1, q2);
    out[2 * i] = q1;
    out[2 * i + 1] = q2;
  }
}
// ... 134 lines not shown
          const int r = (threadIdx.x >> 4) + 16 * ps, cq = threadIdx.x & 15;
          const float4 x = *reinterpret_cast<const float4 *>(w + (long long)(o0 + r) * cin + c0 + 4 * cq);
          tile[r][4 * cq] = x.x;
          tile[r][4 * cq + 1] = x.y;
          tile[r][4 * cq + 2] = x.z;
          tile[r][4 * cq + 3] = x.w;
        }
        __syncthreads();
#pragma unroll
        for (int q = 0; q < 2; ++q) {
          const int idx = threadIdx.x + 256 * q, cl = idx >> 3, o8 = idx & 7;
          float v[8];
#pragma unroll
          for (int k = 0; k < 8; ++k) v[k] = tile[o8 * 8 + k][cl] * scale;
          uint4 q1, q2;
          split2_chunk(v, q1, q2);
          uint4 *dst = wt + SP_NP * ((long long)(c0 + cl) * o8n + (o0 >> 3) + o8);
          dst[0] = q1;
          dst[1] = q2;
        }
      }
    }
    return;
  }
  unsigned short *wk = reinterpret_cast<unsigned short *>(it.wk), *wt = reinterpret_cast<unsigned short *>(it.wt);
  const int cin_pad = it.cin_pad;
  const long long total = (long long)cout * rs * cin_pad;
  if (rs == 1 && cin == cin_pad && (cin % 64) == 0 && (cout % 64) == 0) {
    uint4 *wk4 = reinterpret_cast<uint4 *>(wk);
    for (long long i = (long long)blockIdx.x * 256 + threadIdx.x; i < total / 8; i += (long long)gridDim.x * 256) {
      const float4 lo = reinterpret_cast<const float4 *>(w + i * 8)[0], hi = reinterpret_cast<const float4 *>(w + i * 8)[1];
      wk4[i] = make_uint4(bf16_pack2(lo.x, lo.y), bf16_pack2(lo.z, lo.w), bf16_pack2(hi.x, hi.y), bf16_pack2(hi.z, hi.w));
    }
    if (wt) {
      const int tc = cin / 64, ntiles = (cout / 64) * tc;
      for (int t = blockIdx.x; t < ntiles; t += gridDim.x) {
        const int o0 = (t / tc) * 64, c0 = (t % tc) * 64;
        __syncthreads();
#pragma unroll
        for (int ps = 0; ps < 4; ++ps) {
          const int r = (threadIdx.x >> 4) + 16 * ps, cq = threadIdx.x & 15;
          const float4 x = *reinterpret_cast<const float4 *>(w + (long long)(o0 + r) * cin + c0 + 4 * cq);
          tile[r][4 * cq] = x.x;
          tile[r][4 * cq + 1] = x.y;
          tile[r][4 * cq + 2] = x.z;
          tile[r][4 * cq + 3] = x.w;
        }
        __syncthreads();
#pragma unroll
        for (int q = 0; q < 2; ++q) {
          const int idx = threadIdx.x + 256 * q, cl = idx >> 3, o8 = idx & 7;
          float v[8];
#pragma unroll
          for (int k = 0; k < 8; ++k) v[k] = tile[o8 * 8 + k][cl];
          *reinterpret_cast<uint4 *>(wt + (long long)(c0 + cl) * cout + o0 + o8 * 8) =
              make_uint4(bf16_pack2(v[0], v[1]), bf16_pack2(v[2], v[3]), bf16_pack2(v[4], v[5]), bf16_pack2(v[6], v[7]));
        }
      }
    }
    return;
  }
  for (long long i = (long long)blockIdx.x * 256 + threadIdx.x; i < total; i += (long long)gridDim.x * 256) {
    const int c = (int)(i % cin_pad);
    const long long t = i / cin_pad;
    const int tap = (int)(t % rs), o = (int)(t / rs);
    const float v = c < cin ? w[((long long)o * rs + tap) * cin + c] : 0.f;
    const __bf16 b = (__bf16)v;
    const unsigned short u = __builtin_bit_cast(unsigned short, b);
    wk[i] = u;
    if (wt) wt[((long long)c * rs + tap) * cout + o] = u;
  }
}

typedef float f32x4 __attribute__((ext_vector_type(4)));

#define SPLIT16_ONE(PA, PB)                                                                       \
  _Pragma("unroll") for (int i = 0; i < TM; ++i) _Pragma("unroll") for (int j = 0; j < TN; ++j)   \
      acc[i][j] = __builtin_amdgcn_mfma_f32_16x16x32_f16(av[PA][i], bv[PB][j], acc[i][j], 0, 0, 0);

__device__ __forceinline__ int sp_row_swz(int R) { return ((R >> 1) & 1) | (((R >> 2) & 1) << 2); }

enum AForm : int { A_DMA = 0, A_DY = 1, A_OUT_SP = 2, A_OUT_AFFINE = 3 };
constexpr int BNA_MAX_C = 512;

__device__ __forceinline__ void unpack8(const float4 (&v)[2], float (&o)[8]) {
  o[0] = v[0].x; o[1] = v[0].y; o[2] = v[0].z; o[3] = v[0].w; o[4] = v[1].x; o[5] = v[1].y; o[6] = v[1].z; o[7] = v[1].w;
}

struct DyFormer {
  static constexpr int TABLES = 5;
  __amdgpu_buffer_rsrc_t rs_dz, rs_y;
  float inv_rows, dsc;
  float4 dzv[2][2], yv[2][2];
  float mu[8], is[8], ga[8], sa[8], sb[8];
  static __device__ __forceinline__ void stage(float *t, const IgemmParams &p, int g, int C, int tid) {
    for (int i = tid; i < C; i += 256) {
      const long long gc = (long long)g * C + i;
      t[i] = p.bna_mean[gc];
      t[C + i] = p.bna_invstd[gc];
      t[2 * C + i] = p.bna_gamma[i];
      t[3 * C + i] = p.bna_s1[gc];
      t[4 * C + i] = p.bna_s2[gc];
    }
  }
  __device__ __forceinline__ DyFormer(const IgemmParams &p, long long grow0, long long rows_per_group, int C)
      : rs_dz(make_rsrc(p.bna_dz + grow0 * C, 4ll * rows_per_group * C)), rs_y(make_rsrc(p.bna_y + grow0 * C, 4ll * rows_per_group * C)),
        inv_rows(p.bna_inv_rows), dsc(1.f / *p.a_sinv) {}
  __device__ __forceinline__ void load(int i, unsigned off) {
    dzv[i][0] = buf_ld16(rs_dz, off);
    dzv[i][1] = buf_ld16(rs_dz, off + 16u);
    yv[i][0] = buf_ld16(rs_y, off);
    yv[i][1] = buf_ld16(rs_y, off + 16u);
  }
  __device__ __forceinline__ void consts(const float *kc, int C) {
    ld8(kc, mu);
    ld8(kc + C, is);
    ld8(kc + 2 * C, ga);
    ld8(kc + 3 * C, sa);
    ld8(kc + 4 * C, sb);
  }
  __device__ __forceinline__ void form(int i, bool ok, float (&o)[8]) {
    float d[8], v[8];
    unpack8(dzv[i], d);
    unpack8(yv[i], v);
    bn_dy_chunk(d, v, mu, is, ga, sa, sb, inv_rows, dsc, o, false, mu, mu);
#pragma unroll
    for (int k = 0; k < 8; ++k) o[k] = ok ? o[k] : 0.f;
  }
  __device__ __forceinline__ void store_extra(int, unsigned) {}
};

template <bool AFFINE>
struct OutFormer {
  static constexpr int TABLES = AFFINE ? 4 : 2;
  __amdgpu_buffer_rsrc_t rs_y, rs_r;
  float osc, rsi;
  unsigned short *bits_out;
  float4 yv[2][2], rv[2][2];
  float sc[8], sh[8], rs[8], rh[8];
  unsigned mb[2];
  static __device__ __forceinline__ void stage(float *t, const IgemmParams &p, int g, int C, int tid) {
    for (int i = tid; i < C; i += 256) {
      const long long gc = (long long)g * C + i;
      t[i] = p.fap_scale[gc];
      t[C + i] = p.fap_shift[gc];
      if constexpr (AFFINE) {
        t[2 * C + i] = p.fap_res_scale[gc];
        t[3 * C + i] = p.fap_res_shift[gc];
      }
    }
  }
  __device__ __forceinline__ OutFormer(const IgemmParams &p, long long grow0, long long rows_per_group, int C)
      : rs_y(make_rsrc(p.fap_y + grow0 * C, 4ll * rows_per_group * C)),
        rs_r(make_rsrc(reinterpret_cast<const float *>(p.fap_res) + grow0 * C, 4ll * rows_per_group * C)),
        osc(__uint_as_float(__builtin_amdgcn_readfirstlane(__float_as_uint(p.a_sinv ? 1.f / *p.a_sinv : 1.f)))),
        rsi(__uint_as_float(__builtin_amdgcn_readfirstlane(__float_as_uint((!AFFINE && p.fap_res_sinv) ? *p.fap_res_sinv : 1.f)))),
        bits_out(p.fap_bits ? p.fap_bits + grow0 * (C >> 3) : nullptr) {}
  __device__ __forceinline__ void load(int i, unsigned off) {
    yv[i][0] = buf_ld16(rs_y, off);
    yv[i][1] = buf_ld16(rs_y, off + 16u);
    rv[i][0] = buf_ld16(rs_r, off);
    rv[i][1] = buf_ld16(rs_r, off + 16u);
  }
  __device__ __forceinline__ void consts(const float *kc, int C) {
    ld8(kc, sc);
    ld8(kc + C, sh);
// ... 164 lines not shown
  for (int i = 1; i < b.n; ++i) k += (int)blockIdx.x >= b.it[i].block0;
  wgrad_slab_sum(sh, b.it[k]);
}

__global__ __launch_bounds__(256) void stem_rowwindow_kernel(const float4 *__restrict__ x, uint4 *__restrict__ xw, long long n, int h, int w) {
  const int wo = w >> 1;
  for (long long i = (long long)blockIdx.x * 256 + threadIdx.x; i < n; i += (long long)gridDim.x * 256) {
    const int q = (int)(i & 3);
    const long long t = i >> 2;
    const int ox = (int)(t % wo);
    const long long row = t / wo;
    const int c0 = 2 * ox - 4 + 2 * q;
    float v[8] = {0.f, 0.f, 0.f, 0.f, 0.f, 0.f, 0.f, 0.f};
    if (c0 >= 0 && c0 < w) {
      const float4 a = x[row * w + c0], b = x[row * w + c0 + 1];
      v[0] = a.x; v[1] = a.y; v[2] = a.z; v[3] = a.w; v[4] = b.x; v[5] = b.y; v[6] = b.z; v[7] = b.w;
    }
    uint4 q1, q2;
    split2_chunk(v, q1, q2);
    xw[SP_NP * i] = q1;
    xw[SP_NP * i + 1] = q2;
  }
}

__global__ __launch_bounds__(256) void stem_rowwindow_nchw_kernel(const float *__restrict__ x, uint4 *__restrict__ xw, long long n, int h, int w) {
  const int wo = w >> 1;
  const long long plane = (long long)h * w;
  for (long long i = (long long)blockIdx.x * 256 + threadIdx.x; i < n; i += (long long)gridDim.x * 256) {
    const int q = (int)(i & 3);
    const long long t = i >> 2;
    const int ox = (int)(t % wo);
    const long long row = t / wo;
    const long long img = row / h;
    const int yy = (int)(row - img * h);
    const int c0 = 2 * ox - 4 + 2 * q;
    float v[8] = {0.f, 0.f, 0.f, 0.f, 0.f, 0.f, 0.f, 0.f};
    if (c0 >= 0 && c0 < w) {
      const float *src = x + img * 3 * plane + (long long)yy * w + c0;
      const float2 r = *reinterpret_cast<const float2 *>(src), g = *reinterpret_cast<const float2 *>(src + plane),
                   b = *reinterpret_cast<const float2 *>(src + 2 * plane);
      v[0] = r.x; v[1] = g.x; v[2] = b.x; v[4] = r.y; v[5] = g.y; v[6] = b.y;
    }
    uint4 q1, q2;
    split2_chunk(v, q1, q2);
    xw[SP_NP * i] = q1;
    xw[SP_NP * i + 1] = q2;
  }
}

static int validate_split(const mvg_conv_desc *d) {
  if (validate(d)) return 2;
  MVG_REQUIRE(d->cin % 32 == 0 && d->cout % 32 == 0, "split conv: cin and cout must be multiples of 32 (got %d, %d)", d->cin,
              d->cout);
  MVG_REQUIRE(d->r * d->s <= 32, "split conv: at most 32 filter taps");
  return 0;
}

static int split_tile_rows(int ncols, int taps, long long rows) { return (ncols < 128 && taps > 1 && rows >= 65536) ? 256 : SP_BM; }

struct SplitPlan { int bm, bn, kt_max; long long tiles; bool pipelined; };
static int split_conv_stages(const SplitPlan &pl) { return (pl.pipelined && pl.bn == 128 && pl.bm == SP_BM) ? 2 : 1; }
static SplitPlan split_plan(int ncols, int taps, long long rows, int groups, bool lin, IgemmClass *cls, int ncls) {
  SplitPlan pl;
  pl.bm = lin ? SP_BM : split_tile_rows(ncols, taps, rows);
  pl.bn = ncols >= 128 ? 128 : 64;
  if (lin && pl.bn == 128 && ncls == 1) {
    const long long t128 = (long long)groups * ceil_div(cls[0].rows_per_group, pl.bm) * ceil_div(ncols, 128);
    if (2 * t128 <= compute_cus()) pl.bn = 64;
  }
  pl.tiles = 0, pl.kt_max = 0;
  for (int i = 0; i < ncls; ++i) {
    IgemmClass &c = cls[i];
    c.mtiles_per_group = ceil_div(c.rows_per_group, pl.bm);
    c.KT = ceil_div(c.ktotal, SP_BK);
    c.tile0 = (int)pl.tiles;
    pl.tiles += (long long)groups * c.mtiles_per_group * ceil_div(ncols, pl.bn);
    pl.kt_max = c.KT > pl.kt_max ? c.KT : pl.kt_max;
  }
  pl.pipelined = pl.tiles <= 2LL * compute_cus() || (pl.tiles <= 4LL * compute_cus() && pl.kt_max >= 48);
  return pl;
}

template <bool DGRAD>
static int launch_igemm_split(IgemmParams &p, hipStream_t st, bool lin, int taps, long long rows, AForm af = A_DMA, bool ranged = false) {
  const SplitPlan pl = split_plan(p.ncols, taps, rows, p.groups, lin, p.cls, p.ncls);
  const int bm = pl.bm, bn = pl.bn;
  const bool pipelined = pl.pipelined;
  p.ntiles = ceil_div(p.ncols, bn);
  p.splits = 1;
  p.sk_tiles = 0;
  p.bn_parts = 0;
  for (int i = 0; i < p.ncls; ++i) {
    IgemmClass &c = p.cls[i];
    c.korder = c.ntaps > 1 ? 1 : 0;
    c.per_div = make_fastdiv((unsigned)(c.ntaps > 0 ? c.ntaps : 1));
    c.unit0 = 0;
    c.part0 = p.bn_parts;
    p.bn_parts += c.mtiles_per_group;
    MVG_REQUIRE((c.ntaps >= 1 || (DGRAD && p.bn_part)) && c.ntaps <= 32 && c.ktotal % SP_BK == 0, "split conv: class shape not covered");
  }
  MVG_REQUIRE(pl.tiles < (1LL << 31), "split conv: grid too large");
  if (pl.tiles <= 0) return 0;
  p.nt_out = (!lin && !(DGRAD && p.cls_step == 2)) ? 1 : 0;
  dim3 grid((unsigned)pl.tiles), block(256);
  if (af != A_DMA) {
    MVG_REQUIRE(!lin && bm == SP_BM && p.ntiles == 1 && p.ncls == 1 && DGRAD == (af == A_DY), "split conv: the operand-forming loaders take one column tile");
    if constexpr (DGRAD) {
      if (bn == 128) hipLaunchKernelGGL((igemm_split16_kernel<128, true, false, 2, 1, A_DY>), grid, block, 0, st, p);
      else hipLaunchKernelGGL((igemm_split16_kernel<64, true, false, 2, 1, A_DY>), grid, block, 0, st, p);
      return check_launch("conv_dgrad_split_bnapply");
    } else {
      if (bn == 128 && af == A_OUT_AFFINE) hipLaunchKernelGGL((igemm_split16_kernel<128, false, false, 2, 1, A_OUT_AFFINE>), grid, block, 0, st, p);
      else if (bn == 128) hipLaunchKernelGGL((igemm_split16_kernel<128, false, false, 2, 1, A_OUT_SP>), grid, block, 0, st, p);
      else if (af == A_OUT_AFFINE) hipLaunchKernelGGL((igemm_split16_kernel<64, false, false, 2, 1, A_OUT_AFFINE>), grid, block, 0, st, p);
      else hipLaunchKernelGGL((igemm_split16_kernel<64, false, false, 2, 1, A_OUT_SP>), grid, block, 0, st, p);
      return check_launch("conv_fprop_split_bnapply");
    }
  }
  if (ranged) {
    MVG_REQUIRE(!DGRAD && !lin && p.out_sp && p.out_absmax, "split conv: the range record goes with a forward that stores sp");
    if constexpr (!DGRAD) {
      if (bm == 256) hipLaunchKernelGGL((igemm_split16_ranged_kernel<64, 4>), grid, block, 0, st, p);
      else if (split_conv_stages(pl) == 2) hipLaunchKernelGGL((igemm_split16_ranged_kernel<128, 2, 2>), grid, block, 0, st, p);
      else if (bn == 128) hipLaunchKernelGGL((igemm_split16_ranged_kernel<128>), grid, block, 0, st, p);
      else hipLaunchKernelGGL((igemm_split16_ranged_kernel<64>), grid, block, 0, st, p);
    }
    return check_launch("conv_fprop_split_ranged");
  }
  if (lin) {
    if (bn == 128 && pipelined) hipLaunchKernelGGL((igemm_split16_kernel<128, DGRAD, true, 2, 2>), grid, block, 0, st, p);
    else if (bn == 128) hipLaunchKernelGGL((igemm_split16_kernel<128, DGRAD, true>), grid, block, 0, st, p);
    else if (pipelined) hipLaunchKernelGGL((igemm_split16_kernel<64, DGRAD, true, 2, 2>), grid, block, 0, st, p);
    else hipLaunchKernelGGL((igemm_split16_kernel<64, DGRAD, true>), grid, block, 0, st, p);
  } else if (bm == 256) hipLaunchKernelGGL((igemm_split16_kernel<64, DGRAD, false, 4>), grid, block, 0, st, p);
  else if (split_conv_stages(pl) == 2) hipLaunchKernelGGL((igemm_split16_kernel<128, DGRAD, false, 2, 2>), grid, block, 0, st, p);
  else if (bn == 128) hipLaunchKernelGGL((igemm_split16_kernel<128, DGRAD>), grid, block, 0, st, p);
  else hipLaunchKernelGGL((igemm_split16_kernel<64, DGRAD>), grid, block, 0, st, p);
  return check_launch(DGRAD ? "conv_dgrad_split" : "conv_fprop_split");
}

}

using namespace mvg;

extern "C" {

int mvg_split_f32(const float *x, void *out_sp, int64_t n, float scale, void *stream) {
  MVG_REQUIRE(x && out_sp && n >= 0 && n % 8 == 0, "split_f32: null argument or n %% 8 != 0");
  MVG_REQUIRE(scale > 0.f, "split_f32: scale must be positive (a power of two keeps the round trip exact)");
  if (n == 0) return 0;
  hipStream_t st = (hipStream_t)stream;
  ProfScope ps(MVG_K_LAYOUT, st, 0.0, (4.0 + SP_BYTES) * (double)n);
  long long blocks = (n / 8 + 255) / 256;
  if (blocks > 8192) blocks = 8192;
  hipLaunchKernelGGL(split_f32_kernel, dim3((unsigned)blocks), dim3(256), 0, st, (const float4 *)x, (uint4 *)out_sp, (long long)(n / 8), scale);
  return check_launch("split_f32");
}

int mvg_split_f32_ranged(const float *x, void *out_sp, int64_t n, float scale, uint32_t *range_word, void *stream) {
  MVG_REQUIRE(x && out_sp && range_word && n >= 0 && n % 8 == 0, "split_f32_ranged: null argument or n %% 8 != 0");
  MVG_REQUIRE(scale > 0.f, "split_f32_ranged: scale must be positive (a power of two keeps the round trip exact)");
  if (n == 0) return 0;
  hipStream_t st = (hipStream_t)stream;
  ProfScope ps(MVG_K_LAYOUT, st, 0.0, (4.0 + SP_BYTES) * (double)n);
  long long blocks = (n / 8 + 255) / 256;
  if (blocks > 8192) blocks = 8192;
  hipLaunchKernelGGL(split_f32_ranged_kernel, dim3((unsigned)blocks), dim3(256), 0, st, (const float4 *)x, (uint4 *)out_sp, (long long)(n / 8), scale,
                     (unsigned *)range_word);
  return check_launch("split_f32_ranged");
}

int mvg_merge_sp(const void *x_sp, float *out, int64_t n, float inv_scale, void *stream) {
  MVG_REQUIRE(x_sp && out && n >= 0 && n % 8 == 0, "merge_sp: null argument or n %% 8 != 0");
  if (n == 0) return 0;
  hipStream_t st = (hipStream_t)stream;
  ProfScope ps(MVG_K_LAYOUT, st, 0.0, (4.0 + SP_BYTES) * (double)n);
  long long blocks = (n / 8 + 255) / 256;
  if (blocks > 8192) blocks = 8192;
  hipLaunchKernelGGL(merge_sp_kernel, dim3((unsigned)blocks), dim3(256), 0, st, (const uint4 *)x_sp, (float4 *)out, (long long)(n / 8), inv_scale);
  return check_launch("merge_sp");
}

int mvg_split_weights(const mvg_conv_desc *d, const float *w, void *w_krsc_sp, void *w_crsk_sp, float *stat2, void *items_dev,
                      void *stream) {
  MVG_REQUIRE(d && w && w_krsc_sp && stat2 && items_dev, "split_weights: null argument");
  if (validate_split(d)) return 2;
  hipStream_t st = (hipStream_t)stream;
  WPrepItem it;
  memset(&it, 0, sizeof(it));
  it.w = w;
  it.wk = w_krsc_sp;
  it.wt = w_crsk_sp;
  it.cout = d->cout;
  it.rs = d->r * d->s;
  it.cin = d->cin;
  it.cin_pad = d->cin;
  it.stat = stat2;
  static_assert(sizeof(WPrepItem) <= 64, "WPrepItem grew: update the callers' table record size");
  hipLaunchKernelGGL(wprep_stage_item_kernel, dim3(1), dim3(64), 0, st, it, (WPrepItem *)items_dev);
  if (check_launch("split_weights: staging the table record")) return 1;
  const long long n8 = (long long)d->cout * it.rs * d->cin / 8;
  long long blocks = (n8 + 256 * 8 - 1) / (256 * 8);
  return mvg_weights_prep_batch(items_dev, 1, 1, (int)(blocks < 16 ? 16 : (blocks > 2048 ? 2048 : blocks)), stream);
}

int mvg_weights_prep_batch(const void *items_dev, int n, int mode, int blocks_per_item, void *stream) {
  MVG_REQUIRE(items_dev != nullptr && n > 0 && (mode == 0 || mode == 1) && blocks_per_item >= 0 && blocks_per_item <= 4096,
              "weights_prep_batch: bad arguments");
  hipStream_t st = (hipStream_t)stream;
  ProfScope ps(MVG_K_LAYOUT, st, 0.0, 0.0);
  const unsigned bx = blocks_per_item > 0 ? (unsigned)blocks_per_item : 64u;
  if (mode == 1) {
    hipLaunchKernelGGL(weights_absmax_kernel, dim3(bx > 64 ? bx / 2 : 16, (unsigned)n), dim3(256), 0, st, (const WPrepItem *)items_dev);
    if (check_launch("weights_absmax")) return 1;
  }
  hipLaunchKernelGGL(weights_prep_batch_kernel, dim3(bx, (unsigned)n), dim3(256), 0, st, (const WPrepItem *)items_dev, mode);
  return check_launch("weights_prep_batch");
}

int mvg_conv_stats_partials_split(const mvg_conv_desc *d, int32_t *rows_per_partial) {
  if (validate_split(d)) return -1;
  const long long rows = (long long)d->n * d->ho * d->wo;
  if (rows_per_partial) *rows_per_partial = 64;
  return ceil_div(rows, SP_BM) * 2;
}

struct SplitAffine {
  const float *scale, *shift;
  const void *residual;
  int residual_sp, relu, out_sp;
  int lin;
  float *out_absmax, *out_sinv;
  const float *bias_absmax;
  uint32_t *range_word;
};

struct SplitFwdApply {
  const float *y, *scale, *shift, *res_scale, *res_shift, *res_sinv;
  const void *res;
  uint8_t *bits;
};

static int fprop_split_impl(const mvg_conv_desc *d, const void *x_sp, const float *x_sinv, const void *w_sp, const float *w_sinv,
                            void *y, float *stats, void *stream, const SplitAffine *aff, int stride_w = -1, int pad_w = -1,
                            const SplitFwdApply *fap = nullptr) {
  if (stride_w < 0 && validate_split(d)) return 2;
  IgemmParams p;
  memset(&p, 0, sizeof(p));
  p.a = (const float *)x_sp;
  p.b = (const float *)w_sp;
  p.a_sinv = x_sinv;
  p.b_sinv = w_sinv;
  p.out = (float *)y;
  p.stats = stats;
  if (aff) {
    p.scale = aff->scale;
    p.bias = aff->shift;
    p.addend = (const float *)aff->residual;
    p.addend_sp = aff->residual_sp;
    p.relu = aff->relu;
    p.out_sp = aff->out_sp;
    p.out_absmax = aff->range_word ? (unsigned *)aff->range_word : (unsigned *)aff->out_absmax;
    p.out_sinv = aff->out_sinv;
    p.bias_absmax = aff->bias_absmax;
  }
  if (fap) {
    p.fap_y = fap->y;
    p.fap_scale = fap->scale;
    p.fap_shift = fap->shift;
    p.fap_res = fap->res;
    p.fap_res_scale = fap->res_scale;
    p.fap_res_shift = fap->res_shift;
    p.fap_res_sinv = fap->res_sinv;
    p.fap_bits = (unsigned short *)fap->bits;
  }
  if (fprop_geometry(p, d, SP_BYTES, SP_BYTES, "split conv", stride_w, pad_w)) return 2;
  MVG_REQUIRE(p.rows_per_group * (long long)d->cout < (1ll << 31), "split conv: a group of the output exceeds 2^31 elements");
  const double flops = 2.0 * d->groups * (double)p.rows_per_group * d->cout * d->r * d->s * d->cin * (stride_w >= 0 ? 147.0 / 224.0 : 1.0);
  const double bytes = (double)SP_BYTES * (d->groups * (double)d->n * d->h * d->w * d->cin + (double)d->cout * d->r * d->s * d->cin) +
                       4.0 * d->groups * (double)p.rows_per_group * d->cout +
                       (fap ? 8.0 + 1.0 / 4.0 : 0.0) * d->groups * (double)d->n * d->h * d->w * d->cin;
  const bool lin = d->r == 1 && d->s == 1 && d->h == 1 && d->w == 1;
  ProfScope ps(lin ? MVG_K_LINEAR_FPROP : MVG_K_CONV_FPROP, (hipStream_t)stream, flops, bytes);
  p.stats_partials = ceil_div(p.rows_per_group, SP_BM) * 2;
  return launch_igemm_split<false>(p, (hipStream_t)stream, aff && aff->lin, d->r * d->s, p.rows_per_group,
                                   fap ? (fap->res_scale ? A_OUT_AFFINE : A_OUT_SP) : A_DMA, aff && aff->range_word);
}

int mvg_conv_fprop_split(const mvg_conv_desc *d, const void *x_sp, const float *x_sinv, const void *w_sp, const float *w_sinv, float *y,
                         float *stats, void *stream) {
  return fprop_split_impl(d, x_sp, x_sinv, w_sp, w_sinv, y, stats, stream, nullptr);
}

int mvg_conv_fprop_split_stages(const mvg_conv_desc *d) {
  if (validate_split(d)) return -1;
  IgemmClass c;
  memset(&c, 0, sizeof(c));
  c.rows_per_group = (long long)d->n * d->ho * d->wo;
  c.ktotal = d->r * d->s * d->cin;
  const SplitPlan pl = split_plan(d->cout, d->r * d->s, c.rows_per_group, d->groups, false, &c, 1);
  return split_conv_stages(pl);
}

int mvg_conv_fprop_split_bnapply(const mvg_conv_desc *d, void *out_sp, const float *out_sinv, const float *bn_y, const float *scale,
                                 const float *shift, const void *residual, int residual_sp, const float *res_scale,
                                 const float *res_shift, const float *res_sinv, uint8_t *relu_bits, const void *w_sp,
                                 const float *w_sinv, float *y, float *stats, void *stream) {
  MVG_REQUIRE(d && out_sp && bn_y && scale && shift && residual && w_sp && y, "fprop_split_bnapply: null argument");
  MVG_REQUIRE(d->r == 1 && d->s == 1 && d->stride == 1 && d->pad == 0, "fprop_split_bnapply: 1x1, stride 1, pad 0 only");
  MVG_REQUIRE(d->cout == 64 || d->cout == 128, "fprop_split_bnapply: cout must be 64 or 128 (one column tile; got %d)", d->cout);
  MVG_REQUIRE(d->cin % 32 == 0 && d->cin <= BNA_MAX_C, "fprop_split_bnapply: cin must be a multiple of 32, at most %d (got %d)", BNA_MAX_C,
              d->cin);
  MVG_REQUIRE(residual_sp ? (!res_scale && !res_shift) : (res_scale && res_shift && !res_sinv),
              "fprop_split_bnapply: the residual is an sp identity (no res_scale / res_shift) or fp32 with res_scale and res_shift");
  MVG_REQUIRE((long long)d->n * d->h * d->w * d->cin < (1ll << 29), "fprop_split_bnapply: a group of the input exceeds 2 GiB");
  const SplitFwdApply a = {bn_y, scale, shift, res_scale, res_shift, res_sinv, residual, relu_bits};
  return fprop_split_impl(d, out_sp, out_sinv, w_sp, w_sinv, y, stats, stream, nullptr, -1, -1, &a);
}

int mvg_conv_fprop_split_affine(const mvg_conv_desc *d, const void *x_sp, const float *x_sinv, const void *w_sp, const float *w_sinv,
                                void *out, int out_sp, const float *scale, const float *shift, const void *residual, int residual_sp,
                                int relu, void *stream) {
  MVG_REQUIRE(scale && shift && out, "fprop_split_affine: scale, shift and out are required");
  const SplitAffine a = {scale, shift, residual, residual_sp, relu, out_sp, 0, nullptr, nullptr, nullptr, nullptr};
  return fprop_split_impl(d, x_sp, x_sinv, w_sp, w_sinv, out, nullptr, stream, &a);
}

int mvg_conv_fprop_split_affine_ranged(const mvg_conv_desc *d, const void *x_sp, const float *x_sinv, const void *w_sp, const float *w_sinv,
                                       void *out, int out_sp, const float *scale, const float *shift, const void *residual,
                                       int residual_sp, int relu, uint32_t *range_word, void *stream) {
  MVG_REQUIRE(scale && shift && out, "fprop_split_affine_ranged: scale, shift and out are required");
  MVG_REQUIRE(range_word && out_sp, "fprop_split_affine_ranged: range_word is required and the output must be sp (out_sp != 0)");
  const SplitAffine a = {scale, shift, residual, residual_sp, relu, out_sp, 0, nullptr, nullptr, nullptr, range_word};
  return fprop_split_impl(d, x_sp, x_sinv, w_sp, w_sinv, out, nullptr, stream, &a);
}

struct SplitBnFuse {
  const float *y;
  const uint8_t *bits;
  const float *mean, *invstd, *rscale, *rshift;
  float *part;
  int part_rows;
};

struct SplitBnApply {
  const float *dz, *y, *mean, *invstd, *gamma, *s1, *s2;
  long long rows_per_group;
};

static int dgrad_split_impl(const mvg_conv_desc *d, const void *dy_sp, const float *dy_sinv, const void *w_crsk_sp, const float *w_sinv,
                            float *dx, const float *addend, void *stream, const SplitBnFuse *bnf, const void *relu_mask_sp = nullptr,
                            bool lin_kernel = false, float *out_absmax = nullptr, const SplitBnApply *bna = nullptr) {
  if (validate_split(d)) return 2;
  IgemmParams p;
  memset(&p, 0, sizeof(p));
  p.a = (const float *)dy_sp;
  p.b = (const float *)w_crsk_sp;
  p.a_sinv = dy_sinv;
  p.b_sinv = w_sinv;
  p.out = dx;
  p.addend = addend;
  p.mask = (const float *)relu_mask_sp;
  p.mask_sp = relu_mask_sp != nullptr;
  p.out_absmax = (unsigned *)out_absmax;
  if (bnf) {
    p.bn_y = bnf->y;
    p.bn_bits = bnf->bits;
    p.bn_mean = bnf->mean;
    p.bn_invstd = bnf->invstd;
    p.bn_rscale = bnf->rscale;
    p.bn_rshift = bnf->rshift;
    p.bn_part = bnf->part;
    p.bn_part_rows = bnf->part_rows;
  }
  if (bna) {
    p.bna_dz = bna->dz;
    p.bna_y = bna->y;
    p.bna_mean = bna->mean;
    p.bna_invstd = bna->invstd;
    p.bna_gamma = bna->gamma;
    p.bna_s1 = bna->s1;
    p.bna_s2 = bna->s2;
    p.bna_inv_rows = 1.0f / (float)bna->rows_per_group;
  }
  if (dgrad_geometry(p, d, SP_BYTES, SP_BYTES, "split conv")) return 2;
  MVG_REQUIRE((long long)d->n * d->h * d->w * d->cin < (1ll << 31), "split conv: a group of dx exceeds 2^31 elements");
  const double flops = 2.0 * d->groups * (double)d->n * d->ho * d->wo * d->cout * d->r * d->s * d->cin;
  const double bytes = (double)SP_BYTES * (d->groups * (double)d->n * d->ho * d->wo * d->cout + (double)d->cout * d->r * d->s * d->cin) +
                       (bnf ? 8.25 : 4.0) * d->groups * (double)d->n * d->h * d->w * d->cin +
                       (bna ? 8.0 : 0.0) * d->groups * (double)d->n * d->ho * d->wo * d->cout;
  const bool lin = d->r == 1 && d->s == 1 && d->h == 1 && d->w == 1;
  ProfScope ps(lin ? MVG_K_LINEAR_DGRAD : MVG_K_CONV_DGRAD, (hipStream_t)stream, flops, bytes);
  if (int e = dgrad_classes(p, d, bnf != nullptr, 4, dx, addend, (hipStream_t)stream)) return e;
  if (p.ncls == 0) return 0;
  return launch_igemm_split<true>(p, (hipStream_t)stream, lin_kernel, d->r * d->s, (long long)d->n * d->h * d->w, bna ? A_DY : A_DMA);
}

int mvg_conv_dgrad_split(const mvg_conv_desc *d, const void *dy_sp, const float *dy_sinv, const void *w_crsk_sp, const float *w_sinv,
                         float *dx, const float *addend, const void *relu_mask_sp, void *stream) {
// ... 283 lines not shown
```

rot-mvgaze_amd/csrc/conv_split_igemm.inc:

```
#ifndef MVG_SPLIT_RNG
#error "conv_split_igemm.inc: define MVG_SPLIT_RNG (0 or 1) before including"
#endif

#if MVG_SPLIT_RNG
template <int BN, int WGM = 2, int STAGES = 1>
__global__ __launch_bounds__(256, STAGES == 2 ? 2 : WGM == 4 ? 3 : 4) void igemm_split16_ranged_kernel(IgemmParams p) {
  constexpr bool DGRAD = false, LIN = false;
  constexpr AForm AF = A_DMA;
#else
template <int BN, bool DGRAD, bool LIN = false, int WGM = 2, int STAGES = 1, AForm AF = A_DMA>
__global__ __launch_bounds__(256, STAGES == 2 ? 2 : (DGRAD || WGM == 4 || AF != A_DMA) ? 3 : 4) void igemm_split16_kernel(IgemmParams p) {
#endif
  constexpr int BM = 64 * WGM, WGN = 4 / WGM, NW = 4;
  static_assert(WGM == 2 || (WGM == 4 && BN == 64), "tiles: 128 x BN (2 x 2 waves) or 256 x 64 (4 x 1)");
  static_assert(STAGES == 1 || STAGES == 2, "one LDS stage, or the two-stage pipeline");
  static_assert(AF == A_DMA || (DGRAD == (AF == A_DY) && !LIN && WGM == 2 && STAGES == 1),
                "operand-forming loaders: dy in backward-data, the block output in forward; 128-row tiles, one stage");
  using Former = std::conditional_t<AF == A_DY, DyFormer, OutFormer<AF == A_OUT_AFFINE>>;
  constexpr int WTM = BM / WGM, WTN = BN / WGN;
  constexpr int TM = WTM / 16, TN = WTN / 16;
  constexpr int SLOTS = 4 * SP_NP;
  constexpr int ROWB = 16 * SLOTS, ROWS = BM + BN, STAGE_B = ROWS * ROWB;
  constexpr int NQ = ROWS * SLOTS / 64;
  constexpr int QA = BM * SLOTS / 64;
  constexpr int A_PER = QA / NW, B_PER = (NQ - QA) / NW;
  static_assert(QA % NW == 0 && (NQ - QA) % NW == 0, "whole instructions per wave");
  constexpr int EPI_B = bf16_epilogue_bytes<BM, BN, WGM, DGRAD>();
  constexpr int INFO_OFF = STAGES * STAGE_B > EPI_B ? STAGES * STAGE_B : EPI_B;
  constexpr int BNK_OFF = INFO_OFF + BM * 8;
  constexpr int SMEM_B = BNK_OFF + (AF != A_DMA ? Former::TABLES : 0) * BNA_MAX_C * 4;
  __shared__ __attribute__((aligned(16))) unsigned char smem[SMEM_B];

  const int tid = threadIdx.x;
  const int lane = tid & 63, wave = __builtin_amdgcn_readfirstlane(tid >> 6);
  const int wm = wave / WGN, wn = wave % WGN;
  const int nwg = gridDim.x;
  const int wg_all = p.no_remap ? (int)blockIdx.x : xcd_remap(blockIdx.x, nwg);
  int ci = 0;
  for (int i = 1; i < p.ncls; ++i) ci += wg_all >= p.cls[i].tile0;
  const IgemmClass &c = p.cls[ci];
  const int wg = wg_all - c.tile0;
  const int ntile = wg % p.ntiles;
  const int mt_all = wg / p.ntiles;
  const int g = mt_all / c.mtiles_per_group;
  const int mtile = mt_all - g * c.mtiles_per_group;
  const int KT = c.KT;
  const int ohw = c.out_h * c.out_w;

  uint2 *rowinfo = reinterpret_cast<uint2 *>(smem + INFO_OFF);
  if (tid < BM) {
    const long long m = (long long)mtile * BM + tid;
    const bool ok = m < c.rows_per_group;
    const int mm = ok ? (int)m : 0;
    const int img = (int)fdiv((unsigned)mm, c.ohw_div);
    const int rem = mm - img * ohw;
    const int oy = (int)fdiv((unsigned)rem, c.ow_div), ox = rem - oy * c.out_w;
    const int y0 = DGRAD ? oy + c.cls_cy : oy * p.stride - p.pad;
    const int x0 = DGRAD ? ox + c.cls_cx : ox * p.stride_w - p.pad_w;
    const unsigned base = (unsigned)(img * p.src_img_stride * SP_BYTES) + (unsigned)((y0 * p.src_w + x0) * p.src_c) * (unsigned)SP_BYTES;
    unsigned msk = 0;
    for (int t = 0; t < c.ntaps; ++t) {
      const int fr = (int)fdiv((unsigned)t, c.tap_ns_div), fs = t - fr * c.tap_ns;
      const int iy = DGRAD ? y0 - fr : y0 + fr;
      const int ix = DGRAD ? x0 - fs : x0 + fs;
      msk |= (unsigned)(((unsigned)iy < (unsigned)p.src_h) & ((unsigned)ix < (unsigned)p.src_w)) << t;
    }
    rowinfo[tid] = make_uint2(base, ok ? msk : 0u);
  }
  if constexpr (AF != A_DMA) Former::stage(reinterpret_cast<float *>(smem + BNK_OFF), p, g, p.src_c, tid);
  __syncthreads();
  unsigned a_base[A_PER], a_vmask[A_PER], b_base[B_PER];
#pragma unroll
  for (int i = 0; i < A_PER; ++i) {
    const int sl = (wave + NW * i) * 64 + lane;
    const int row = sl / SLOTS, j = (sl % SLOTS) ^ sp_row_swz(row);
    const uint2 ri = rowinfo[row];
    a_base[i] = ri.x + 16u * (unsigned)j;
    a_vmask[i] = ri.y;
  }
#pragma unroll
  for (int i = 0; i < B_PER; ++i) {
    const int sl = (wave + NW * (A_PER + i)) * 64 + lane - BM * SLOTS;
    const int row = sl / SLOTS, j = (sl % SLOTS) ^ sp_row_swz(row);
    const int n = ntile * BN + row;
    b_base[i] = pred_off(((unsigned)n * (unsigned)p.b_row_len) * (unsigned)SP_BYTES + 16u * (unsigned)j, n < p.ncols);
  }
  const __amdgpu_buffer_rsrc_t rs_a =
      make_rsrc(reinterpret_cast<const char *>(p.a) + (long long)g * p.imgs_per_group * p.src_img_stride * SP_BYTES, p.a_group_bytes);
  const __amdgpu_buffer_rsrc_t rs_b = make_rsrc(p.b, p.b_bytes);
  typedef __attribute__((address_space(3))) void *lds_vp;

  auto issue = [&](int kt, int stage_off) {
    int kstart = kt * SP_BK;
    if (c.korder) {
      const int cblk = (int)fdiv((unsigned)kt, c.per_div), rem = kt - cblk * c.ntaps;
      kstart = (rem << p.src_c_shift) + cblk * SP_BK;
    }
    const int ks = __builtin_amdgcn_readfirstlane(kstart);
    const int tap_u = c.ntaps > 1 ? (ks >> p.src_c_shift) : 0;
    const int chb = ks - (tap_u << p.src_c_shift);
    const int fru = (int)fdiv((unsigned)tap_u, c.tap_ns_div), fsu = tap_u - fru * c.tap_ns;
    const int disp = (fru * p.src_w + fsu) * p.src_c;
    const unsigned sdelta = (unsigned)(((DGRAD ? -disp : disp) + chb) * SP_BYTES);
    unsigned kb = (unsigned)ks * (unsigned)SP_BYTES;
    if (DGRAD) {
      const int btap = (c.tap_r0 + p.tap_step * fru) * p.s + c.tap_s0 + p.tap_step * fsu;
      kb = (unsigned)(btap * p.src_c + chb) * (unsigned)SP_BYTES;
    }
    if constexpr (AF == A_DMA) {
#pragma unroll
      for (int i = 0; i < A_PER; ++i) {
        const bool ok = ((a_vmask[i] >> tap_u) & 1u) != 0u;
        __builtin_amdgcn_raw_ptr_buffer_load_lds(rs_a, (lds_vp)(smem + stage_off + (wave + NW * i) * 1024), 16, (int)pred_off(a_base[i] + sdelta, ok), 0, 0, 0);
      }
    }
#pragma unroll
    for (int i = 0; i < B_PER; ++i)
      __builtin_amdgcn_raw_ptr_buffer_load_lds(rs_b, (lds_vp)(smem + stage_off + (wave + NW * (A_PER + i)) * 1024), 16, (int)(b_base[i] + kb), 0, 0, 0);
  };

  f32x4 acc[TM][TN];
#pragma unroll
  for (int i = 0; i < TM; ++i)
#pragma unroll
    for (int j = 0; j < TN; ++j)
#pragma unroll
      for (int e = 0; e < 4; ++e) acc[i][j][e] = 0.f;

  const int cc_l = lane >> 4;
  int a_off[TM][SP_NP], b_off[TN][SP_NP];
#pragma unroll
  for (int i = 0; i < TM; ++i) {
    const int R = wm * WTM + i * 16 + (lane & 15);
#pragma unroll
    for (int pc = 0; pc < SP_NP; ++pc) a_off[i][pc] = R * ROWB + (((2 * cc_l + pc) ^ sp_row_swz(R)) << 4);
  }
#pragma unroll
  for (int j = 0; j < TN; ++j) {
    const int R = wn * WTN + j * 16 + (lane & 15);
#pragma unroll
    for (int pc = 0; pc < SP_NP; ++pc) b_off[j][pc] = (BM + R) * ROWB + (((2 * cc_l + pc) ^ sp_row_swz(R)) << 4);
  }

  auto load_frags = [&](const unsigned char *stage, f16x8 (&av)[SP_NP][TM], f16x8 (&bv)[SP_NP][TN]) {
#pragma unroll
    for (int pc = 0; pc < SP_NP; ++pc) {
#pragma unroll
      for (int i = 0; i < TM; ++i) av[pc][i] = *reinterpret_cast<const f16x8 *>(stage + a_off[i][pc]);
#pragma unroll
      for (int j = 0; j < TN; ++j) bv[pc][j] = *reinterpret_cast<const f16x8 *>(stage + b_off[j][pc]);
    }
  };
  auto products = [&](const f16x8 (&av)[SP_NP][TM], const f16x8 (&bv)[SP_NP][TN]) { SPLIT16_ONE(0, 1) SPLIT16_ONE(1, 0) SPLIT16_ONE(0, 0) };
  if constexpr (AF != A_DMA) {
    const int C = p.src_c;
    const int a_cc = tid & 3, a_r0 = tid >> 2;
    const long long grow0 = (long long)g * c.rows_per_group;
    Former f(p, grow0, c.rows_per_group, C);
    uint4 *a_out = reinterpret_cast<uint4 *>(const_cast<float *>(p.a)) + grow0 * C / 4;
    bool a_ok[2];
    unsigned a_goff[2];
#pragma unroll
    for (int i = 0; i < 2; ++i) {
      const long long m = (long long)mtile * BM + a_r0 + 64 * i;
      a_ok[i] = m < c.rows_per_group;
      a_goff[i] = pred_off((unsigned)m * (unsigned)C * 4u + 32u * (unsigned)a_cc, a_ok[i]);
    }
    auto a_load = [&](int kt) {
#pragma unroll
      for (int i = 0; i < 2; ++i) f.load(i, a_goff[i] + 128u * (unsigned)kt);
    };
    constexpr bool PREFETCH = BN == 64;
    if (PREFETCH) a_load(0);
    for (int kt = 0; kt < KT; ++kt) {
      issue(kt, 0);
      if (!PREFETCH) a_load(kt);
      uint4 q[2][SP_NP];
      f.consts(reinterpret_cast<const float *>(smem + BNK_OFF) + kt * SP_BK + a_cc * 8, C);
#pragma unroll
      for (int i = 0; i < 2; ++i) {
        float o[8];
        f.form(i, a_ok[i], o);
        split2_chunk(o, q[i][0], q[i][1]);
        const int R = a_r0 + 64 * i;
#pragma unroll
        for (int pc = 0; pc < SP_NP; ++pc)
          *reinterpret_cast<uint4 *>(smem + R * ROWB + (((2 * a_cc + pc) ^ sp_row_swz(R)) << 4)) = q[i][pc];
      }
      asm volatile("s_waitcnt vmcnt(0)" ::: "memory");
      __syncthreads();
#pragma unroll
      for (int i = 0; i < 2; ++i)
        if (a_ok[i]) {
          const unsigned off = a_goff[i] + 128u * (unsigned)kt;
          uint4 *dst = a_out + (off >> 4);
          dst[0] = q[i][0];
          dst[1] = q[i][1];
          f.store_extra(i, off);
        }
      if (PREFETCH && kt + 1 < KT) a_load(kt + 1);
      {
        f16x8 av[SP_NP][TM], bv[SP_NP][TN];
        load_frags(smem, av, bv);
        products(av, bv);
      }
      __syncthreads();
    }
  } else if constexpr (STAGES == 1) {
    for (int kt = 0; kt < KT; ++kt) {
      issue(kt, 0);
      asm volatile("s_waitcnt vmcnt(0)" ::: "memory");
      __syncthreads();
      {
        f16x8 av[SP_NP][TM], bv[SP_NP][TN];
        load_frags(smem, av, bv);
        products(av, bv);
      }
      __syncthreads();
    }
  } else {
    constexpr int G = A_PER + B_PER;
    if (KT > 0) issue(0, 0);
    if (KT > 1) {
      issue(1, STAGE_B);
      asm volatile("s_waitcnt vmcnt(%0)\n\ts_barrier" ::"n"(G) : "memory");
    } else {
      asm volatile("s_waitcnt vmcnt(0)\n\ts_barrier" ::: "memory");
    }
    f16x8 a0[SP_NP][TM], b0[SP_NP][TN], a1[SP_NP][TM], b1[SP_NP][TN];
    load_frags(smem, a0, b0);
    int cur = 0;
    auto step = [&](int kt, const f16x8 (&ca)[SP_NP][TM], const f16x8 (&cb)[SP_NP][TN], f16x8 (&na)[SP_NP][TM], f16x8 (&nb)[SP_NP][TN]) {
      if (kt + 1 < KT) {
        asm volatile("s_waitcnt vmcnt(0) lgkmcnt(0)\n\ts_barrier" ::: "memory");
        if (kt + 2 < KT) issue(kt + 2, cur);
        cur ^= STAGE_B;
        load_frags(smem + cur, na, nb);
      }
      products(ca, cb);
    };
    for (int kt = 0; kt < KT; kt += 2) {
      step(kt, a0, b0, a1, b1);
      if (kt + 1 < KT) step(kt + 1, a1, b1, a0, b0);
    }
    __syncthreads();
  }
#if MVG_SPLIT_RNG
  bf16_epilogue<BM, BN, WGM, DGRAD, true, WGM, true, DGRAD, LIN, WGN, false, true>(p, c, acc, reinterpret_cast<unsigned short *>(smem), tid, g, mtile,
                                                                                     ntile);
#else
  bf16_epilogue<BM, BN, WGM, DGRAD, true, WGM, true, DGRAD, LIN, WGN>(p, c, acc, reinterpret_cast<unsigned short *>(smem), tid, g, mtile, ntile);
#endif
}
```

rot-mvgaze_amd/ops.py:

```python
from __future__ import annotations

import ctypes as C
from typing import Optional

import torch

from ._lib import ConvDesc, K_FAMILIES, ProfEntry, check, lib

Tensor = torch.Tensor


def _p(t: Optional[Tensor]):
    if t is None:
        return None
    assert t.is_cuda and t.dtype in _PTR_DTYPES, (t.device, t.dtype)
    return t.data_ptr()


_PTR_DTYPES = frozenset((torch.float32, torch.int32, torch.uint8, torch.int16, torch.bfloat16, torch.float16))
_workspaces = {}
_MAX_WORKSPACES = 8
_raw_stream = getattr(torch._C, "_cuda_getCurrentRawStream", None)


# ... 186 lines not shown
    return t is not None and t.dtype == torch.float16


def split_f32(x: Tensor, scale: float = 1.0) -> Tensor:
    assert x.dtype == torch.float32 and x.is_contiguous() and x.shape[-1] % 8 == 0
    out = sp_empty(*x.shape, device=x.device)
    check(lib().mvg_split_f32(_p(x), _p(out), x.numel(), float(scale), _s()), "split_f32")
    out.sinv = None if scale == 1.0 else torch.full((1,), 1.0 / scale, dtype=torch.float32, device=x.device)
    return out


def split_f32_ranged(x: Tensor, range_word: Tensor, scale: float = 1.0) -> Tensor:
    assert x.dtype == torch.float32 and x.is_contiguous() and x.shape[-1] % 8 == 0
    assert range_word.dtype == torch.int32 and range_word.numel() == 1
    out = sp_empty(*x.shape, device=x.device)
    check(lib().mvg_split_f32_ranged(_p(x), _p(out), x.numel(), float(scale), _p(range_word), _s()), "split_f32_ranged")
    out.sinv = None if scale == 1.0 else torch.full((1,), 1.0 / scale, dtype=torch.float32, device=x.device)
    return out


def merge_sp(x: Tensor) -> Tensor:
    assert is_sp(x) and x.is_contiguous() and x.shape[-1] == 8 and x.shape[-2] == 2
    out = torch.empty(sp_shape(x), dtype=torch.float32, device=x.device)
    sinv = getattr(x, "sinv", None)
    check(lib().mvg_merge_sp(_p(x), _p(out), out.numel(), float(sinv.item()) if sinv is not None else 1.0, _s()), "merge_sp")
    return out


_items_scratch = {}


def split_weights(d: ConvDesc, w: Tensor, need_transposed: bool = True):
    assert w.dtype == torch.float32 and w.is_cuda
    rs = d.r * d.s
    wk = sp_empty(d.cout, rs * d.cin, device=w.device)
    wt = sp_empty(d.cin, rs * d.cout, device=w.device) if need_transposed else None
    stat = torch.empty(2, dtype=torch.float32, device=w.device)
    items = torch.empty(64, dtype=torch.uint8, device=w.device)
    check(lib().mvg_split_weights(C.byref(d), _p(w), _p(wk), _p(wt), _p(stat), _p(items), _s()), "split_weights")
    wk.sinv = stat[1:2]
    if wt is not None:
        wt.sinv = stat[1:2]
    return wk, wt


def weights_prep_batch(table: Tensor, n: int, mode: int, blocks_per_item: int = 0):
    assert table.is_cuda and table.dtype == torch.int64 and table.is_contiguous() and table.shape == (n, 6)
    check(lib().mvg_weights_prep_batch(C.c_void_p(table.data_ptr()), n, mode, blocks_per_item, _s()), "weights_prep_batch")


def conv_stats_partials_split(d: ConvDesc):
    rpp = C.c_int32(0)
    n = lib().mvg_conv_stats_partials_split(C.byref(d), C.byref(rpp))
    if n < 0:
        check(1, "conv_stats_partials_split")
    return n, rpp.value


def conv_fprop_split(d: ConvDesc, x_sp: Tensor, w_sp: Tensor, y: Tensor, stats: Optional[Tensor] = None):
    check(lib().mvg_conv_fprop_split(C.byref(d), _p(x_sp), _sinv(x_sp), _p(w_sp), _sinv(w_sp), _p(y), _p(stats), _s()), "conv_fprop_split")


def conv_fprop_split_stages(d: ConvDesc) -> int:
    n = lib().mvg_conv_fprop_split_stages(C.byref(d))
    if n < 0:
        check(1, "conv_fprop_split_stages")
    return n


def conv_dgrad_split_stages(d: ConvDesc, fused_reduce: bool = False) -> int:
    n = lib().mvg_conv_dgrad_split_stages(C.byref(d), int(fused_reduce))
    if n < 0:
        check(1, "conv_dgrad_split_stages")
    return n


def conv_wgrad_split_tile(d: ConvDesc):
    bm, bn, incr = C.c_int32(0), C.c_int32(0), C.c_int32(0)
    if lib().mvg_conv_wgrad_split_tile(C.byref(d), C.byref(bm), C.byref(bn), C.byref(incr)) != 0:
        check(1, "conv_wgrad_split_tile")
    return bm.value, bn.value, bool(incr.value)


def conv_fprop_split_bnapply(d: ConvDesc, out_sp: Tensor, bn_y, scale, shift, residual, w_sp: Tensor, y: Tensor,
                             stats: Optional[Tensor] = None, residual_affine=None, bits: Optional[Tensor] = None):
    assert bits is None or (bits.dtype == torch.uint8 and bits.numel() == d.groups * d.n * d.h * d.w * d.cin // 4)
    rs, rh = residual_affine if residual_affine is not None else (None, None)
    res_sp = is_sp(residual)
    check(lib().mvg_conv_fprop_split_bnapply(C.byref(d), _p(out_sp), _sinv(out_sp), _p(bn_y), _p(scale), _p(shift), _p(residual), int(res_sp),
                                             _p(rs), _p(rh), _sinv(residual) if res_sp else None, _p(bits), _p(w_sp), _sinv(w_sp), _p(y),
                                             _p(stats), _s()), "conv_fprop_split_bnapply")


def conv_fprop_split_affine(d: ConvDesc, x_sp: Tensor, w_sp: Tensor, out: Tensor, scale: Tensor, shift: Tensor,
                            residual: Optional[Tensor], relu: bool):
    assert getattr(residual, "sinv", None) is None, "conv_fprop_split_affine: the residual is read unscaled"
    check(lib().mvg_conv_fprop_split_affine(C.byref(d), _p(x_sp), _sinv(x_sp), _p(w_sp), _sinv(w_sp), _p(out), int(is_sp(out)), _p(scale),
                                            _p(shift), _p(residual), int(is_sp(residual)), int(relu), _s()), "conv_fprop_split_affine")


def conv_fprop_split_affine_ranged(d: ConvDesc, x_sp: Tensor, w_sp: Tensor, out: Tensor, scale: Tensor, shift: Tensor,
                                   residual: Optional[Tensor], relu: bool, range_word: Tensor):
    assert getattr(residual, "sinv", None) is None, "conv_fprop_split_affine_ranged: the residual is read unscaled"
    assert is_sp(out) and range_word.dtype == torch.int32 and range_word.numel() == 1
    check(lib().mvg_conv_fprop_split_affine_ranged(C.byref(d), _p(x_sp), _sinv(x_sp), _p(w_sp), _sinv(w_sp), _p(out), 1, _p(scale), _p(shift),
                                                   _p(residual), int(is_sp(residual)), int(relu), _p(range_word), _s()),
          "conv_fprop_split_affine_ranged")


def conv_dgrad_split(d: ConvDesc, dy_sp: Tensor, wt_sp: Tensor, dx: Tensor, addend: Optional[Tensor] = None,
                     relu_mask_sp: Optional[Tensor] = None):
    assert relu_mask_sp is None or is_sp(relu_mask_sp)
    check(lib().mvg_conv_dgrad_split(C.byref(d), _p(dy_sp), _sinv(dy_sp), _p(wt_sp), _sinv(wt_sp), _p(dx), _p(addend), _p(relu_mask_sp),
                                     _s()), "conv_dgrad_split")


def stem_rowwindow_split(x_nhwc4: Tensor) -> Tensor:
    G, N, H, W, C = x_nhwc4.shape
    assert C == 4 and W % 2 == 0 and x_nhwc4.dtype == torch.float32 and x_nhwc4.is_contiguous()
    xw = sp_empty(G, N, H, W // 2, 32, device=x_nhwc4.device)
    check(lib().mvg_stem_rowwindow_split(_p(x_nhwc4), _p(xw), G * N, H, W, _s()), "stem_rowwindow_split")
    xw.sinv = None
    return xw


def stem_rowwindow_split_nchw(x_nchw: Tensor, out: Tensor):
    B, Cc, H, W = x_nchw.shape
    assert Cc == 3 and W % 2 == 0 and x_nchw.dtype == torch.float32 and x_nchw.is_contiguous() and is_sp(out) and out.is_contiguous()
    assert sp_shape(out) == (B, H, W // 2, 32)
    check(lib().mvg_stem_rowwindow_split_nchw(_p(x_nchw), _p(out), B, H, W, _s()), "stem_rowwindow_split_nchw")


def stem_fprop_split(d: ConvDesc, xw: Tensor, w_sp: Tensor, y: Tensor, stats: Optional[Tensor]):
    check(lib().mvg_stem_fprop_split(C.byref(d), _p(xw), _p(w_sp), _sinv(w_sp), _p(y), _p(stats), _s()), "stem_fprop_split")


def stem_wgrad_split(d: ConvDesc, xw: Tensor, dy_sp: Tensor, dw_rw: Tensor, accumulate: bool = False):
    splits, ws = _wgrad_slabs(lib().mvg_stem_wgrad_splits_split, "stem_wgrad_splits_split", d, d.cout * 224, xw.device)
    check(lib().mvg_stem_wgrad_split(C.byref(d), _p(xw), _p(dy_sp), _sinv(dy_sp), _p(dw_rw), _p(ws), splits, int(accumulate), _s()),
          "stem_wgrad_split")


def bn_relu_maxpool_bwd_reduce_split(g_pooled, argmax, y, mean, invstd, scale, shift, groups, n_per_group, h, w, c, ho, wo, s1, s2,
                                     dgamma, dbeta, accumulate, mx, gamma=None, dy_sinv=None):
    n = lib().mvg_bn_bwd_workspace_floats(groups, n_per_group * h * w, c)
    ws = torch.empty(n, dtype=torch.float32, device=y.device)
    check(lib().mvg_bn_relu_maxpool_bwd_reduce_split(_p(g_pooled), _p(argmax), _p(y), _p(mean), _p(invstd), _p(scale), _p(shift), groups,
                                                     n_per_group, h, w, c, ho, wo, _p(s1), _p(s2), _p(dgamma), _p(dbeta), int(accumulate),
                                                     _p(ws), _p(mx), _p(gamma), _p(dy_sinv), _s()), "bn_relu_maxpool_bwd_reduce_split")


def bn_relu_maxpool_bwd_apply_split(g_pooled, argmax, y, mean, invstd, gamma, scale, shift, s1, s2, groups, n_per_group, h, w, c, ho, wo,
                                    dy_sp, mx, dy_sinv=None):
    ready = dy_sinv is not None
    dy_sp.sinv = dy_sinv if ready else torch.empty(1, dtype=torch.float32, device=y.device)
    check(lib().mvg_bn_relu_maxpool_bwd_apply_split(_p(g_pooled), _p(argmax), _p(y), _p(mean), _p(invstd), _p(gamma), _p(scale), _p(shift),
                                                    _p(s1), _p(s2), groups, n_per_group, h, w, c, ho, wo, _p(dy_sp), _p(mx), _p(dy_sp.sinv),
                                                    int(ready), _s()), "bn_relu_maxpool_bwd_apply_split")


def stem_rowwindow_bf16(x_nchw: Tensor, out: Tensor):
    B, Cc, H, W = x_nchw.shape
    assert Cc == 3 and W % 4 == 0 and x_nchw.dtype == torch.float32 and x_nchw.is_contiguous()
    assert out.dtype == torch.bfloat16 and out.shape == (B, H, W // 4, 64) and out.is_contiguous()
    check(lib().mvg_stem_rowwindow_bf16(_p(x_nchw), _p(out), B, H, W, _s()), "stem_rowwindow_bf16")


def stem_fprop_bf16(d: ConvDesc, xw: Tensor, w_fold: Tensor, y: Tensor, stats: Optional[Tensor]):
    check(lib().mvg_stem_fprop_bf16(C.byref(d), _p(xw), _p(w_fold), _p(y), _p(stats), _s()), "stem_fprop_bf16")


def stem_wgrad_bf16(d: ConvDesc, xw: Tensor, dy: Tensor, dw_fold: Tensor, accumulate: bool = False):
    splits, ws = _wgrad_slabs(lib().mvg_stem_wgrad_splits_bf16, "stem_wgrad_splits_bf16", d, 2 * d.cout * 448, xw.device)
    check(lib().mvg_stem_wgrad_bf16(C.byref(d), _p(xw), _p(dy), _p(dw_fold), _p(ws), splits, int(accumulate), _s()), "stem_wgrad_bf16")
# ... 508 lines not shown
```

Measured before the change: 1677 samples/s.

## Add wide 64x256 tile form to fuse BN-apply into 256-column 1x1 forward convs

Extends the fused BN-apply/residual/ReLU-into-next-conv forward path to consumers with 256 output channels and up to 1024 input channels. It uses a new 64x256 tile (1x4 waves) with a two-pass column epilogue and larger per-channel LDS tables. This removes the standalone bn_apply_split kernel and its activation round-trip for those ResNet-50 block transitions. The cost is lower occupancy (launch bounds of 2 for the affine form), more LDS, and extra code for zeroing the unused stats partial slot.

```diff
diff --git a/include/rotmvgaze.h b/include/rotmvgaze.h
--- a/include/rotmvgaze.h
+++ b/include/rotmvgaze.h
@@ -394,6 +394,10 @@
                                  const float *shift, const void *residual, int residual_sp, const float *res_scale,
                                  const float *res_shift, const float *res_sinv, uint8_t *relu_bits, const void *w_sp,
                                  const float *w_sinv, float *y, float *stats, void *stream);
+int mvg_conv_fprop_split_bnapply_wide(const mvg_conv_desc *d, void *out_sp, const float *out_sinv, const float *bn_y, const float *scale,
+                                      const float *shift, const void *residual, int residual_sp, const float *res_scale,
+                                      const float *res_shift, const float *res_sinv, uint8_t *relu_bits, const void *w_sp,
+                                      const float *w_sinv, float *y, float *stats, void *stream);
 int mvg_stem_rowwindow_split(const float *x_nhwc4, void *xw_sp, int64_t images, int h, int w, void *stream);
 int mvg_stem_rowwindow_split_nchw(const float *x_nchw, void *xw_sp, int64_t images, int h, int w, void *stream);
 int mvg_stem_fprop_split(const mvg_conv_desc *d, const void *xw_sp, const void *w_sp, const float *w_sinv, float *y, float *stats,
diff --git a/rot-mvgaze_amd/_lib.py b/rot-mvgaze_amd/_lib.py
--- a/rot-mvgaze_amd/_lib.py
+++ b/rot-mvgaze_amd/_lib.py
@@ -131,6 +131,7 @@
     "mvg_conv_fprop_split_stages": (_I, [_D]),
     "mvg_conv_dgrad_split_stages": (_I, [_D, _I]),
     "mvg_conv_fprop_split_bnapply": (_I, [_D] + [_P] * 6 + [_I] + [_P] * 9),
+    "mvg_conv_fprop_split_bnapply_wide": (_I, [_D] + [_P] * 6 + [_I] + [_P] * 9),
     "mvg_conv_wgrad_splits_split": (_I, [_D]),
     "mvg_conv_wgrad_split_tile": (_I, [_D, C.POINTER(C.c_int32), C.POINTER(C.c_int32), C.POINTER(C.c_int32)]),
     "mvg_conv_wgrad_split": (_I, [_D, _P, _P, _P, _P, _P, _I, _I, _P]),
diff --git a/rot-mvgaze_amd/backbone.py b/rot-mvgaze_amd/backbone.py
--- a/rot-mvgaze_amd/backbone.py
+++ b/rot-mvgaze_amd/backbone.py
@@ -53,6 +53,29 @@
     return [(a.convs[-1].name, b.convs[0].name) for a, b in zip(spec.blocks[:-1], spec.blocks[1:])
             if bn_apply_fprop_eligible(a.convs[-1], b.convs[0], split=on, trained=training,
                                        single_stage=True if single_stage is None else single_stage(b.convs[0]))]
+
+
+BN_APPLY_FPROP_WIDE_COUT = 256
+BN_APPLY_FPROP_WIDE_MAX_CIN = 1024
+
+
+def bn_apply_fprop_wide_eligible(producer: ConvSpec, consumer: ConvSpec, *, split: bool, trained: bool, residual: bool = True,
+                                 relu: bool = True, single_stage: bool = True, residual_affine: bool = False) -> bool:
+    return bool(split and trained and residual and relu and single_stage and not residual_affine
+                and consumer.k == 1 and consumer.stride == 1 and consumer.pad == 0 and consumer.cout == BN_APPLY_FPROP_WIDE_COUT
+                and consumer.cin == producer.cout and consumer.cin % 32 == 0 and consumer.cin <= BN_APPLY_FPROP_WIDE_MAX_CIN)
+
+
+def bn_apply_fprop_wide_may_plan(groups: int, rows_per_group: int) -> bool:
+    return groups * ((rows_per_group + 127) // 128) * 2 > 16
+
+
+def bn_apply_fprop_wide_pairs(spec: BackboneSpec, *, split: bool = True, bf16: bool = False, training: bool = True, enabled: bool = True,
+                              single_stage: Optional[Callable[[ConvSpec], bool]] = None) -> List[tuple]:
+    on = enabled and split and not bf16
+    return [(a.convs[-1].name, b.convs[0].name) for a, b in zip(spec.blocks[:-1], spec.blocks[1:])
+            if bn_apply_fprop_wide_eligible(a.convs[-1], b.convs[0], split=on, trained=training, residual_affine=a.downsample is not None,
+                                            single_stage=True if single_stage is None else single_stage(b.convs[0]))]
 
 
 class GradSink:
@@ -146,6 +169,7 @@
     residual: Optional[Tensor]
     residual_affine: Optional[tuple]
     bits: Optional[Tensor]
+    wide: bool = False
 
 
 class _PendingDy(NamedTuple):
@@ -218,6 +242,7 @@
         self.fuse_bn_split = True
         self.fuse_bn_apply_dgrad = True
         self.fuse_bn_apply_fprop = True
+        self.fuse_bn_apply_fprop_wide = True
         self.stem_rowwindow = True
         self.split_eval = True
         self.split_eval_guard: Optional[str] = None
@@ -502,7 +527,8 @@
                 ops.stem_fprop_split(d, x, w, y, stats)
             elif pending_apply is not None:
                 p = pending_apply
-                ops.conv_fprop_split_bnapply(d, x, p.y, p.scale, p.shift, p.residual, w, y, stats, p.residual_affine, p.bits)
+                launch = ops.conv_fprop_split_bnapply_wide if p.wide else ops.conv_fprop_split_bnapply
+                launch(d, x, p.y, p.scale, p.shift, p.residual, w, y, stats, p.residual_affine, p.bits)
             else:
                 ops.conv_fprop_split(d, x, w, y, stats)
         else:
@@ -528,12 +554,17 @@
             out = ops.sp_empty(G, d.n, d.ho, d.wo, c.cout, device=y.device)
             out.sinv = call.act_sinv[c.name]
             want_bits = keep and relu and residual is not None
-            if (next_conv is not None and self.fuse_bn_apply_fprop
-                    and bn_apply_fprop_eligible(c, next_conv, split=family is Family.SPLIT, trained=call.training,
-                                                residual=residual is not None, relu=relu)
+            narrow = (next_conv is not None and self.fuse_bn_apply_fprop
+                      and bn_apply_fprop_eligible(c, next_conv, split=family is Family.SPLIT, trained=call.training,
+                                                  residual=residual is not None, relu=relu))
+            wide = (next_conv is not None and self.fuse_bn_apply_fprop_wide
+                    and bn_apply_fprop_wide_eligible(c, next_conv, split=family is Family.SPLIT, trained=call.training,
+                                                     residual=residual is not None, relu=relu,
+                                                     residual_affine=residual_affine is not None))
+            if ((narrow or (wide and bn_apply_fprop_wide_may_plan(G, rows)))
                     and ops.conv_fprop_split_stages(ConvDesc.make(G, d.n, d.ho, d.wo, next_conv.cin, next_conv.cout, 1, 1, 0)) == 1):
                 bits = torch.empty(G * rows * c.cout // 4, dtype=torch.uint8, device=y.device) if want_bits else None
-                return out, bits, _Apply(y, scale, shift, residual, residual_affine, bits)
+                return out, bits, _Apply(y, scale, shift, residual, residual_affine, bits, wide)
             bits = ops.bn_apply_split(y, scale, shift, residual, relu, out, G, rows, c.cout, residual_affine, want_bits=want_bits)
             return out, bits, None
         out = torch.empty_like(y) if keep else y
diff --git a/rot-mvgaze_amd/csrc/bf16_tile.h b/rot-mvgaze_amd/csrc/bf16_tile.h
--- a/rot-mvgaze_amd/csrc/bf16_tile.h
+++ b/rot-mvgaze_amd/csrc/bf16_tile.h
@@ -47,14 +47,16 @@
 }
 
 template <int BM, int BN, int WGM, bool DGRAD, bool F32IO, int PASSES = 1, bool ACC16 = false, bool BNF = false, bool LIN = false, int WGN = 2,
-          bool AFF = false, bool RNG = false, class AccT>
+          bool AFF = false, bool RNG = false, int CP = 1, class AccT>
 __device__ __forceinline__ void bf16_epilogue(const IgemmParams &p, const IgemmClass &c, AccT &acc,
                                               unsigned short *smem, int tid, int g, int mtile, int ntile) {
   constexpr int NT = WGM * WGN * 64;
   constexpr int WTM = BM / WGM, WTN = BN / WGN;
   constexpr int TS = ACC16 ? 16 : 32, NE = ACC16 ? 4 : 16;
   constexpr int TM = WTM / TS, TN = WTN / TS;
-  constexpr int LDO = BN + 4;
+  constexpr int BNC = BN / CP;
+  constexpr int LDO = BNC + 4;
+  static_assert(CP == 1 || (F32IO && !DGRAD && !BNF && !AFF && WGN % CP == 0), "bf16_epilogue: column passes are a forward form of the split kernels");
   const int lane = tid & 63, wave = tid >> 6;
   const int wm = wave / WGN, wn = wave % WGN;
   const int li = ACC16 ? (lane & 15) : (lane & 31), lh = ACC16 ? (lane >> 4) : (lane >> 5);
@@ -143,7 +145,7 @@
   float *out_f = p.out + (long long)g * gelems;
   const float *add_f = p.addend ? p.addend + (long long)g * gelems : nullptr;
   const float *mask_f = p.mask ? p.mask + (long long)g * gelems : nullptr;
-  constexpr int CV = BN / 8;
+  constexpr int CV = BNC / 8;
   const bool bnf = BNF && DGRAD && p.bn_part != nullptr;
   bool quad = false;
   if constexpr (F32IO && DGRAD && !LIN) quad = !p.mask && (p.ncols % BN) == 0;
@@ -173,23 +175,25 @@
     }
   }
 #pragma unroll
-  for (int ph = 0; ph < PASSES; ++ph) {
-  if (PASSES > 1 && ph > 0) __syncthreads();
-  if (wm / (WGM / PASSES) == ph) {
+  for (int pp = 0; pp < PASSES * CP; ++pp) {
+  const int ph = pp / CP, cph = pp % CP;
+  const int wnc = CP == 1 ? wn : wn % (WGN / CP);
+  if (PASSES * CP > 1 && pp > 0) __syncthreads();
+  if (wm / (WGM / PASSES) == ph && (CP == 1 || wn / (WGN / CP) == cph)) {
 #pragma unroll
     for (int i = 0; i < TM; ++i)
 #pragma unroll
       for (int j = 0; j < TN; ++j)
 #pragma unroll
         for (int e = 0; e < NE; ++e)
-          ot[((wm % (WGM / PASSES)) * WTM + i * TS + erow(e)) * LDO + wn * WTN + j * TS + li] = acc[i][j][e];
+          ot[((wm % (WGM / PASSES)) * WTM + i * TS + erow(e)) * LDO + wnc * WTN + j * TS + li] = acc[i][j][e];
   }
   __syncthreads();
   auto store_rows = [&](int it) {
     const int v = tid + it * NT;
     const int rl = v / CV, cv = v - rl * CV;
     const int r = ph * PR + rl;
-    const int col = ntile * BN + cv * 8;
+    const int col = ntile * BN + cph * BNC + cv * 8;
     const int off = rowoff[r];
     if (off < 0 || col >= p.ncols) return;
     const float4 lo = *reinterpret_cast<const float4 *>(ot + rl * LDO + cv * 8);
@@ -451,12 +455,12 @@
   bool plain4 = false;
   if constexpr (F32IO && !LIN) plain4 = p.nt_out && !p.scale && !p.bias && !p.addend && !p.mask && !p.out_sp && !bnf && !p.relu;
   if (plain4) {
-    constexpr int CV4 = BN / 4;
+    constexpr int CV4 = BNC / 4;
 #pragma unroll
     for (int it = 0; it < PR * CV4 / NT; ++it) {
       const int v = tid + it * NT;
       const int rl = v / CV4, c4 = v - rl * CV4;
-      const int col = ntile * BN + c4 * 4;
+      const int col = ntile * BN + cph * BNC + c4 * 4;
       const int off = rowoff[ph * PR + rl];
       if (off < 0 || col >= p.ncols) continue;
       const float4 q = *reinterpret_cast<const float4 *>(ot + rl * LDO + c4 * 4);
diff --git a/rot-mvgaze_amd/csrc/conv_split.hip b/rot-mvgaze_amd/csrc/conv_split.hip
--- a/rot-mvgaze_amd/csrc/conv_split.hip
+++ b/rot-mvgaze_amd/csrc/conv_split.hip
@@ -240,6 +240,8 @@
 
 enum AForm : int { A_DMA = 0, A_DY = 1, A_OUT_SP = 2, A_OUT_AFFINE = 3 };
 constexpr int BNA_MAX_C = 512;
+constexpr int BNA_WIDE_MAX_C = 1024;
+constexpr int SP_WIDE_BM = 64, SP_WIDE_BN = 256;
 
 __device__ __forceinline__ void unpack8(const float4 (&v)[2], float (&o)[8]) {
   o[0] = v[0].x; o[1] = v[0].y; o[2] = v[0].z; o[3] = v[0].w; o[4] = v[1].x; o[5] = v[1].y; o[6] = v[1].z; o[7] = v[1].w;
@@ -570,8 +572,15 @@
 }
 
 template <bool DGRAD>
-static int launch_igemm_split(IgemmParams &p, hipStream_t st, bool lin, int taps, long long rows, AForm af = A_DMA, bool ranged = false) {
-  const SplitPlan pl = split_plan(p.ncols, taps, rows, p.groups, lin, p.cls, p.ncls);
+static int launch_igemm_split(IgemmParams &p, hipStream_t st, bool lin, int taps, long long rows, AForm af = A_DMA, bool ranged = false,
+                              bool wide = false) {
+  SplitPlan pl = split_plan(p.ncols, taps, rows, p.groups, lin, p.cls, p.ncls);
+  if (wide) {
+    MVG_REQUIRE(!DGRAD && af != A_DMA && !lin && p.ncls == 1 && p.ncols == SP_WIDE_BN, "split conv: the wide form is a forming forward with 256 columns");
+    pl.bm = SP_WIDE_BM, pl.bn = SP_WIDE_BN;
+    p.cls[0].mtiles_per_group = ceil_div(p.cls[0].rows_per_group, pl.bm);
+    pl.tiles = (long long)p.groups * p.cls[0].mtiles_per_group;
+  }
   const int bm = pl.bm, bn = pl.bn;
   const bool pipelined = pl.pipelined;
   p.ntiles = ceil_div(p.ncols, bn);
@@ -592,7 +601,14 @@
   p.nt_out = (!lin && !(DGRAD && p.cls_step == 2)) ? 1 : 0;
   dim3 grid((unsigned)pl.tiles), block(256);
   if (af != A_DMA) {
-    MVG_REQUIRE(!lin && bm == SP_BM && p.ntiles == 1 && p.ncls == 1 && DGRAD == (af == A_DY), "split conv: the operand-forming loaders take one column tile");
+    MVG_REQUIRE(!lin && (bm == SP_BM || wide) && p.ntiles == 1 && p.ncls == 1 && DGRAD == (af == A_DY), "split conv: the operand-forming loaders take one column tile");
+    if constexpr (!DGRAD) {
+      if (wide) {
+        if (af == A_OUT_AFFINE) hipLaunchKernelGGL((igemm_split16_kernel<256, false, false, 1, 1, A_OUT_AFFINE>), grid, block, 0, st, p);
+        else hipLaunchKernelGGL((igemm_split16_kernel<256, false, false, 1, 1, A_OUT_SP>), grid, block, 0, st, p);
+        return check_launch("conv_fprop_split_bnapply_wide");
+      }
+    }
     if constexpr (DGRAD) {
       if (bn == 128) hipLaunchKernelGGL((igemm_split16_kernel<128, true, false, 2, 1, A_DY>), grid, block, 0, st, p);
       else hipLaunchKernelGGL((igemm_split16_kernel<64, true, false, 2, 1, A_DY>), grid, block, 0, st, p);
@@ -727,6 +743,7 @@
   const float *y, *scale, *shift, *res_scale, *res_shift, *res_sinv;
   const void *res;
   uint8_t *bits;
+  bool wide;
 };
 
 static int fprop_split_impl(const mvg_conv_desc *d, const void *x_sp, const float *x_sinv, const void *w_sp, const float *w_sinv,
@@ -772,7 +789,7 @@
   ProfScope ps(lin ? MVG_K_LINEAR_FPROP : MVG_K_CONV_FPROP, (hipStream_t)stream, flops, bytes);
   p.stats_partials = ceil_div(p.rows_per_group, SP_BM) * 2;
   return launch_igemm_split<false>(p, (hipStream_t)stream, aff && aff->lin, d->r * d->s, p.rows_per_group,
-                                   fap ? (fap->res_scale ? A_OUT_AFFINE : A_OUT_SP) : A_DMA, aff && aff->range_word);
+                                   fap ? (fap->res_scale ? A_OUT_AFFINE : A_OUT_SP) : A_DMA, aff && aff->range_word, fap && fap->wide);
 }
 
 int mvg_conv_fprop_split(const mvg_conv_desc *d, const void *x_sp, const float *x_sinv, const void *w_sp, const float *w_sinv, float *y,
@@ -802,7 +819,23 @@
   MVG_REQUIRE(residual_sp ? (!res_scale && !res_shift) : (res_scale && res_shift && !res_sinv),
               "fprop_split_bnapply: the residual is an sp identity (no res_scale / res_shift) or fp32 with res_scale and res_shift");
   MVG_REQUIRE((long long)d->n * d->h * d->w * d->cin < (1ll << 29), "fprop_split_bnapply: a group of the input exceeds 2 GiB");
-  const SplitFwdApply a = {bn_y, scale, shift, res_scale, res_shift, res_sinv, residual, relu_bits};
+  const SplitFwdApply a = {bn_y, scale, shift, res_scale, res_shift, res_sinv, residual, relu_bits, false};
+  return fprop_split_impl(d, out_sp, out_sinv, w_sp, w_sinv, y, stats, stream, nullptr, -1, -1, &a);
+}
+
+int mvg_conv_fprop_split_bnapply_wide(const mvg_conv_desc *d, void *out_sp, const float *out_sinv, const float *bn_y, const float *scale,
+                                      const float *shift, const void *residual, int residual_sp, const float *res_scale,
+                                      const float *res_shift, const float *res_sinv, uint8_t *relu_bits, const void *w_sp,
+                                      const float *w_sinv, float *y, float *stats, void *stream) {
+  MVG_REQUIRE(d && out_sp && bn_y && scale && shift && residual && w_sp && y, "fprop_split_bnapply_wide: null argument");
+  MVG_REQUIRE(d->r == 1 && d->s == 1 && d->stride == 1 && d->pad == 0, "fprop_split_bnapply_wide: 1x1, stride 1, pad 0 only");
+  MVG_REQUIRE(d->cout == SP_WIDE_BN, "fprop_split_bnapply_wide: cout must be 256 (one 256-column tile; got %d)", d->cout);
+  MVG_REQUIRE(d->cin % 32 == 0 && d->cin <= BNA_WIDE_MAX_C, "fprop_split_bnapply_wide: cin must be a multiple of 32, at most %d (got %d)",
+              BNA_WIDE_MAX_C, d->cin);
+  MVG_REQUIRE(residual_sp ? (!res_scale && !res_shift) : (res_scale && res_shift && !res_sinv),
+              "fprop_split_bnapply_wide: the residual is an sp identity (no res_scale / res_shift) or fp32 with res_scale and res_shift");
+  MVG_REQUIRE((long long)d->n * d->h * d->w * d->cin < (1ll << 29), "fprop_split_bnapply_wide: a group of the input exceeds 2 GiB");
+  const SplitFwdApply a = {bn_y, scale, shift, res_scale, res_shift, res_sinv, residual, relu_bits, true};
   return fprop_split_impl(d, out_sp, out_sinv, w_sp, w_sinv, y, stats, stream, nullptr, -1, -1, &a);
 }
 
diff --git a/rot-mvgaze_amd/csrc/conv_split_igemm.inc b/rot-mvgaze_amd/csrc/conv_split_igemm.inc
--- a/rot-mvgaze_amd/csrc/conv_split_igemm.inc
+++ b/rot-mvgaze_amd/csrc/conv_split_igemm.inc
@@ -9,13 +9,15 @@
   constexpr AForm AF = A_DMA;
 #else
 template <int BN, bool DGRAD, bool LIN = false, int WGM = 2, int STAGES = 1, AForm AF = A_DMA>
-__global__ __launch_bounds__(256, STAGES == 2 ? 2 : (DGRAD || WGM == 4 || AF != A_DMA) ? 3 : 4) void igemm_split16_kernel(IgemmParams p) {
+__global__ __launch_bounds__(256, (STAGES == 2 || (WGM == 1 && AF == A_OUT_AFFINE)) ? 2 : (DGRAD || WGM == 4 || AF != A_DMA) ? 3 : 4)
+    void igemm_split16_kernel(IgemmParams p) {
 #endif
   constexpr int BM = 64 * WGM, WGN = 4 / WGM, NW = 4;
-  static_assert(WGM == 2 || (WGM == 4 && BN == 64), "tiles: 128 x BN (2 x 2 waves) or 256 x 64 (4 x 1)");
+  static_assert(WGM == 2 || (WGM == 4 && BN == 64) || (WGM == 1 && BN == 256 && AF != A_DMA),
+                "tiles: 128 x BN (2 x 2 waves), 256 x 64 (4 x 1), or 64 x 256 (1 x 4: the operand-forming loaders' wide form)");
   static_assert(STAGES == 1 || STAGES == 2, "one LDS stage, or the two-stage pipeline");
-  static_assert(AF == A_DMA || (DGRAD == (AF == A_DY) && !LIN && WGM == 2 && STAGES == 1),
-                "operand-forming loaders: dy in backward-data, the block output in forward; 128-row tiles, one stage");
+  static_assert(AF == A_DMA || (DGRAD == (AF == A_DY) && !LIN && (WGM == 2 || WGM == 1) && STAGES == 1),
+                "operand-forming loaders: dy in backward-data, the block output in forward; 128- or 64-row tiles, one stage");
   using Former = std::conditional_t<AF == A_DY, DyFormer, OutFormer<AF == A_OUT_AFFINE>>;
   constexpr int WTM = BM / WGM, WTN = BN / WGN;
   constexpr int TM = WTM / 16, TN = WTN / 16;
@@ -25,10 +27,11 @@
   constexpr int QA = BM * SLOTS / 64;
   constexpr int A_PER = QA / NW, B_PER = (NQ - QA) / NW;
   static_assert(QA % NW == 0 && (NQ - QA) % NW == 0, "whole instructions per wave");
-  constexpr int EPI_B = bf16_epilogue_bytes<BM, BN, WGM, DGRAD>();
+  constexpr int EPI_CP = WGM == 1 ? 2 : 1;
+  constexpr int EPI_B = bf16_epilogue_bytes<BM, BN / EPI_CP, WGM, DGRAD>();
   constexpr int INFO_OFF = STAGES * STAGE_B > EPI_B ? STAGES * STAGE_B : EPI_B;
   constexpr int BNK_OFF = INFO_OFF + BM * 8;
-  constexpr int SMEM_B = BNK_OFF + (AF != A_DMA ? Former::TABLES : 0) * BNA_MAX_C * 4;
+  constexpr int SMEM_B = BNK_OFF + (AF != A_DMA ? Former::TABLES : 0) * (WGM == 1 ? BNA_WIDE_MAX_C : BNA_MAX_C) * 4;
   __shared__ __attribute__((aligned(16))) unsigned char smem[SMEM_B];
 
   const int tid = threadIdx.x;
@@ -158,27 +161,28 @@
     const long long grow0 = (long long)g * c.rows_per_group;
     Former f(p, grow0, c.rows_per_group, C);
     uint4 *a_out = reinterpret_cast<uint4 *>(const_cast<float *>(p.a)) + grow0 * C / 4;
-    bool a_ok[2];
-    unsigned a_goff[2];
-#pragma unroll
-    for (int i = 0; i < 2; ++i) {
+    constexpr int AR = BM / 64;
+    bool a_ok[AR];
+    unsigned a_goff[AR];
+#pragma unroll
+    for (int i = 0; i < AR; ++i) {
       const long long m = (long long)mtile * BM + a_r0 + 64 * i;
       a_ok[i] = m < c.rows_per_group;
       a_goff[i] = pred_off((unsigned)m * (unsigned)C * 4u + 32u * (unsigned)a_cc, a_ok[i]);
     }
     auto a_load = [&](int kt) {
 #pragma unroll
-      for (int i = 0; i < 2; ++i) f.load(i, a_goff[i] + 128u * (unsigned)kt);
+      for (int i = 0; i < AR; ++i) f.load(i, a_goff[i] + 128u * (unsigned)kt);
     };
-    constexpr bool PREFETCH = BN == 64;
+    constexpr bool PREFETCH = BN == 64 || WGM == 1;
     if (PREFETCH) a_load(0);
     for (int kt = 0; kt < KT; ++kt) {
       issue(kt, 0);
       if (!PREFETCH) a_load(kt);
-      uint4 q[2][SP_NP];
+      uint4 q[AR][SP_NP];
       f.consts(reinterpret_cast<const float *>(smem + BNK_OFF) + kt * SP_BK + a_cc * 8, C);
 #pragma unroll
-      for (int i = 0; i < 2; ++i) {
+      for (int i = 0; i < AR; ++i) {
         float o[8];
         f.form(i, a_ok[i], o);
         split2_chunk(o, q[i][0], q[i][1]);
@@ -190,7 +194,7 @@
       asm volatile("s_waitcnt vmcnt(0)" ::: "memory");
       __syncthreads();
 #pragma unroll
-      for (int i = 0; i < 2; ++i)
+      for (int i = 0; i < AR; ++i)
         if (a_ok[i]) {
           const unsigned off = a_goff[i] + 128u * (unsigned)kt;
           uint4 *dst = a_out + (off >> 4);
@@ -249,6 +253,15 @@
   bf16_epilogue<BM, BN, WGM, DGRAD, true, WGM, true, DGRAD, LIN, WGN, false, true>(p, c, acc, reinterpret_cast<unsigned short *>(smem), tid, g, mtile,
                                                                                      ntile);
 #else
-  bf16_epilogue<BM, BN, WGM, DGRAD, true, WGM, true, DGRAD, LIN, WGN>(p, c, acc, reinterpret_cast<unsigned short *>(smem), tid, g, mtile, ntile);
+  if constexpr (WGM == 1) {
+    bf16_epilogue<BM, BN, WGM, DGRAD, true, WGM, true, DGRAD, LIN, WGN, false, false, EPI_CP>(p, c, acc, reinterpret_cast<unsigned short *>(smem), tid,
+                                                                                                g, mtile, ntile);
+    if (!DGRAD && p.stats && mtile == c.mtiles_per_group - 1 && mtile + 1 < p.stats_partials) {
+      float *st = p.stats + (((long long)g * p.stats_partials + mtile + 1) * 2) * p.ncols;
+      for (int col = tid; col < 2 * p.ncols; col += 256) st[col] = 0.f;
+    }
+  } else {
+    bf16_epilogue<BM, BN, WGM, DGRAD, true, WGM, true, DGRAD, LIN, WGN>(p, c, acc, reinterpret_cast<unsigned short *>(smem), tid, g, mtile, ntile);
+  }
 #endif
 }
diff --git a/rot-mvgaze_amd/ops.py b/rot-mvgaze_amd/ops.py
--- a/rot-mvgaze_amd/ops.py
+++ b/rot-mvgaze_amd/ops.py
@@ -292,14 +292,25 @@
     return bm.value, bn.value, bool(incr.value)
 
 
-def conv_fprop_split_bnapply(d: ConvDesc, out_sp: Tensor, bn_y, scale, shift, residual, w_sp: Tensor, y: Tensor,
-                             stats: Optional[Tensor] = None, residual_affine=None, bits: Optional[Tensor] = None):
+def _conv_fprop_split_bnapply(entry: str, d: ConvDesc, out_sp: Tensor, bn_y, scale, shift, residual, w_sp: Tensor, y: Tensor,
+                              stats: Optional[Tensor], residual_affine, bits: Optional[Tensor]):
     assert bits is None or (bits.dtype == torch.uint8 and bits.numel() == d.groups * d.n * d.h * d.w * d.cin // 4)
     rs, rh = residual_affine if residual_affine is not None else (None, None)
     res_sp = is_sp(residual)
-    check(lib().mvg_conv_fprop_split_bnapply(C.byref(d), _p(out_sp), _sinv(out_sp), _p(bn_y), _p(scale), _p(shift), _p(residual), int(res_sp),
-                                             _p(rs), _p(rh), _sinv(residual) if res_sp else None, _p(bits), _p(w_sp), _sinv(w_sp), _p(y),
-                                             _p(stats), _s()), "conv_fprop_split_bnapply")
+    check(getattr(lib(), "mvg_" + entry)(C.byref(d), _p(out_sp), _sinv(out_sp), _p(bn_y), _p(scale), _p(shift), _p(residual), int(res_sp),
+                                         _p(rs), _p(rh), _sinv(residual) if res_sp else None, _p(bits), _p(w_sp), _sinv(w_sp), _p(y),
+                                         _p(stats), _s()), entry)
+
+
+def conv_fprop_split_bnapply(d: ConvDesc, out_sp: Tensor, bn_y, scale, shift, residual, w_sp: Tensor, y: Tensor,
+                             stats: Optional[Tensor] = None, residual_affine=None, bits: Optional[Tensor] = None):
+    _conv_fprop_split_bnapply("conv_fprop_split_bnapply", d, out_sp, bn_y, scale, shift, residual, w_sp, y, stats, residual_affine, bits)
+
+
+def conv_fprop_split_bnapply_wide(d: ConvDesc, out_sp: Tensor, bn_y, scale, shift, residual, w_sp: Tensor, y: Tensor,
+                                  stats: Optional[Tensor] = None, residual_affine=None, bits: Optional[Tensor] = None):
+    _conv_fprop_split_bnapply("conv_fprop_split_bnapply_wide", d, out_sp, bn_y, scale, shift, residual, w_sp, y, stats, residual_affine,
+                              bits)
 
 
 def conv_fprop_split_affine(d: ConvDesc, x_sp: Tensor, w_sp: Tensor, out: Tensor, scale: Tensor, shift: Tensor,
```

Result: slower. 1651 samples/s (-1.5%).
